# AaronWatters/contourist

Hardware: AMD Instinct MI355X
Metric: Mvoxels/s isosurface extraction on 512^3 fp32 grid (higher is better)
Workload: dtype f32

## Files before the change

contourist_amd/csrc/cx_post.h:

```cpp
#pragma once
#include <vector>

#include "cx_ctx.h"
#include "cx_dev.h"

struct cx_post_state {
    cx_buf<uint8_t> pts, prio, rep, tri, alive, parent, parent2, tkeys, tvals, flags, scan, blocksums, pts_out, tri_out, comp, misc;
    cx_buf<uint8_t> keys_out, keys_tmp, told, cls, bnd;
    cx_buf<uint8_t> ever;
    bool keys_valid = false;
    cx_buf<uint8_t> vflip;
    bool keys_edge = false, orient_live = false, vflip_valid = false;
    uint32_t orient_nt = 0;
    bool shard_mesh = false;
    double corner[3] = {1.0, 1.0, 1.0};
    uint64_t gen = 0;
    cx_buf<uint8_t> nrm[2], nrm_tmp, smap;
    int nrm_cur = 0;
    bool simplified = false, carried = false, smap_valid = false;
    bool clipped = false;
    uint32_t smap_n = 0;
    uint64_t capped_gen = 0;
    bool capped() const { return capped_gen != 0 && capped_gen == gen; }
    struct {
        bool open = false;
        uint32_t nv2 = 0, nt2 = 0;
        uint32_t nt_in = 0;
        uint32_t n1 = 0, n4 = 0, ncand = 0;
    } shard;
    cx_buf<uint8_t> mpairs, msegs, mtris, mmid, mtime, mnext;
    cx_buf<uint8_t> msegs2, mtris2, mtime2;
    cx_buf<uint8_t> meflags, metflag, menew, mecnt, medesc, me_pts, me_tri;
    void* me_pinned = nullptr;
    bool meflags_clean = false;
    uint32_t mbin_t[257] = {0}, mbin_s[257] = {0};
    double mt_lo = 0.0, mt_inv_width = 0.0;
    double mt_maxdur = 0.0, ms_maxdur = 0.0;
    bool msorted = false;
    std::vector<int64_t> me_off;
    int64_t nv_out = 0, nt_out = 0;
    int64_t ms_out = 0, mt_out = 0;
};

int cxp_state(cx_ctx* ctx, cx_post_state** out);

static inline u64 cxp_edge_table_size(size_t n) {
    u64 s = 1024;
    while (s < (5 * (u64)n) / 4 + 16) s <<= 1;
    return s;
}

int cxp_scan(cx_ctx* ctx, cx_post_state* S, const uint32_t* in, uint32_t* out, uint32_t n, uint32_t* total_dev);

int cxp_orient_pick(cx_ctx* ctx, const int32_t* tri, uint32_t nt, const double* pts, u64* parent, u64* comp, const uint32_t* keys,
                    const uint8_t* cls, uint32_t* clist, uint32_t* misc);
int cxp_orient_decide(cx_ctx* ctx, int32_t* tri, uint32_t nt, const double* pts, const u64* parent, u64* comp, const uint32_t* clist,
                      uint32_t* misc, bool wind, uint32_t* ncomp);

void cxp_iota64(hipStream_t st, u64* a, uint32_t n);
void cxp_fill64(hipStream_t st, u64* a, size_t n, u64 v);
void cxp_count_alive(hipStream_t st, const uint8_t* alive, uint32_t nt, uint32_t* counter);
void cxp_alive_u32(hipStream_t st, const uint8_t* alive, uint32_t nt, uint32_t* out);
void cxp_scan_sums(hipStream_t st, uint32_t* sums, uint32_t nb, uint32_t* total);
```

contourist_amd/csrc/cx_post.hip:

```cpp
#include <algorithm>
#include <cmath>
#include <cstring>
#include <new>
#include <string>
#include <vector>

#include "cx_post.h"

void cx_post_free(cx_ctx* ctx) {
    if (!ctx->post) return;
    cx_post_state* S = ctx->post;
    if (S->me_pinned) (void)hipHostFree(S->me_pinned);
    delete S;
    ctx->post = nullptr;
}

__global__ void cxp_k_iota64(u64* a, uint32_t n) {
    const uint32_t i = blockIdx.x * blockDim.x + threadIdx.x;
    if (i < n) a[i] = (u64)i;
}
__global__ void cxp_k_fill64(u64* a, size_t n, u64 v) {
    for (size_t i = blockIdx.x * (size_t)blockDim.x + threadIdx.x; i < n; i += (size_t)gridDim.x * blockDim.x) a[i] = v;
}
__global__ void cxp_k_jump(u64* parent, uint32_t n, uint32_t* changed) {
    const uint32_t i = blockIdx.x * blockDim.x + threadIdx.x;
    if (i >= n) return;
    u64 w = parent[i];
    uint32_t p = (uint32_t)w;
    if (p == i) return;
    bool moved = false;
#pragma unroll 1
    for (int hop = 0; hop < 3; hop++) {
        const u64 wp = parent[p];
        const uint32_t pp = (uint32_t)wp;
        if (pp == p) break;
        w = ((((w >> 32) ^ (wp >> 32)) & 1ULL) << 32) | (u64)pp;
        p = pp;
        moved = true;
    }
    if (moved) {
        parent[i] = w;
        *changed = 1u;
    }
}

#define CXP_SCAN_BLOCK 1024u
__global__ __launch_bounds__(256) void cxp_k_scan_blocks(const uint32_t* in, uint32_t* out, uint32_t* sums, uint32_t n) {
    __shared__ uint32_t s[256];
    const uint32_t base = blockIdx.x * CXP_SCAN_BLOCK + threadIdx.x * 4u;
    uint32_t v[4], t = 0;
#pragma unroll
    for (int k = 0; k < 4; k++) {
        v[k] = (base + k < n) ? in[base + k] : 0u;
        t += v[k];
    }
    s[threadIdx.x] = t;
    __syncthreads();
    for (uint32_t o = 1; o < 256; o <<= 1) {
        const uint32_t x = (threadIdx.x >= o) ? s[threadIdx.x - o] : 0u;
        __syncthreads();
        s[threadIdx.x] += x;
        __syncthreads();
    }
    uint32_t run = s[threadIdx.x] - t;
#pragma unroll
    for (int k = 0; k < 4; k++) {
        if (base + k < n) out[base + k] = run;
        run += v[k];
    }
    if (threadIdx.x == 255) sums[blockIdx.x] = s[255];
}
#define CXP_SUMS_PER_THREAD 16u
__device__ __forceinline__ void cxp_scan_sums_body(uint32_t* sums, uint32_t nb, uint32_t* total, unsigned long long* total64);
__global__ __launch_bounds__(1024) void cxp_k_scan_sums2(uint32_t* sums_a, uint32_t na, uint32_t* total_a, uint32_t* sums_b, uint32_t nb, uint32_t* total_b) {
    if (blockIdx.x == 0) cxp_scan_sums_body(sums_a, na, total_a, nullptr);
    else cxp_scan_sums_body(sums_b, nb, total_b, nullptr);
}
__global__ __launch_bounds__(1024) void cxp_k_scan_sums(uint32_t* sums, uint32_t nb, uint32_t* total, unsigned long long* total64) {
    cxp_scan_sums_body(sums, nb, total, total64);
}
__device__ __forceinline__ void cxp_scan_sums_body(uint32_t* sums, uint32_t nb, uint32_t* total, unsigned long long* total64) {
    __shared__ uint32_t s[1024];
    uint32_t carry = 0;
    unsigned long long wide = 0;
    for (uint32_t base = 0; base < nb; base += 1024u * CXP_SUMS_PER_THREAD) {
        const uint32_t i0 = base + threadIdx.x * CXP_SUMS_PER_THREAD;
        uint32_t v[CXP_SUMS_PER_THREAD], t = 0;
#pragma unroll
        for (uint32_t k = 0; k < CXP_SUMS_PER_THREAD; k++) {
            v[k] = (i0 + k < nb) ? sums[i0 + k] : 0u;
            t += v[k];
        }
        s[threadIdx.x] = t;
        __syncthreads();
        for (uint32_t o = 1; o < 1024; o <<= 1) {
            const uint32_t x = (threadIdx.x >= o) ? s[threadIdx.x - o] : 0u;
            __syncthreads();
            s[threadIdx.x] += x;
            __syncthreads();
        }
        uint32_t run = carry + s[threadIdx.x] - t;
#pragma unroll
        for (uint32_t k = 0; k < CXP_SUMS_PER_THREAD; k++) {
            if (i0 + k < nb) sums[i0 + k] = run;
            run += v[k];
        }
        const uint32_t passtot = s[1023];
        __syncthreads();
        carry += passtot;
        wide += (unsigned long long)passtot;
    }
    if (threadIdx.x == 0) {
        *total = carry;
        if (total64) *total64 = wide;
    }
}
__global__ void cxp_k_scan_add(uint32_t* out, const uint32_t* sums, uint32_t n) {
    const uint32_t i = blockIdx.x * blockDim.x + threadIdx.x;
    if (i < n) out[i] += sums[i / CXP_SCAN_BLOCK];
}

struct cxp_origin3 {
    double o[3];
};
template <int DT>
__global__ void cxp_k_vertices_f64(const cx_grid_ref A, const double* __restrict__ A64, uint32_t n1, uint32_t n2, cx_fdiv dplane, cx_fdiv drow,
                                   double value, const cx_vrec* __restrict__ verts, uint32_t nv, double* pts, uint32_t* prio, cxp_origin3 org) {
    const uint32_t v = blockIdx.x * blockDim.x + threadIdx.x;
    if (v >= nv) return;
    const uint32_t key = verts[v].x;
    const uint32_t lin = key >> 3, d = key & 7u;
    const uint32_t plane = n1 * n2;
    const uint32_t i = cx_div(lin, dplane);
    const uint32_t r = lin - i * plane;
    const uint32_t j = cx_div(r, drow);
    const uint32_t k = r - j * n2;
    const uint32_t lin2 = lin + ((d & 4u) ? plane : 0u) + ((d & 2u) ? n2 : 0u) + (d & 1u);
    const double f0 = A64 ? A64[lin] : (double)cx_sample<DT>(A, lin), f1 = A64 ? A64[lin2] : (double)cx_sample<DT>(A, lin2);
    const bool owner_low = !(f0 > f1);
    const double flow = owner_low ? f0 : f1, fhigh = owner_low ? f1 : f0;
    double ratio = 0.5;
    const double den = 1.0 * (fhigh - flow);
    if (!(fabs(den) <= 1e-8)) ratio = (value - flow) / den;
    const double q[3] = {(double)i + org.o[0], (double)j + org.o[1], (double)k + org.o[2]};
    const uint32_t db[3] = {(d >> 2) & 1u, (d >> 1) & 1u, d & 1u};
#pragma unroll
    for (int a = 0; a < 3; a++) {
        const double low = owner_low ? q[a] : q[a] + (double)db[a];
        const double high = owner_low ? q[a] + (double)db[a] : q[a];
        pts[(size_t)v * 3 + a] = low + ratio * (high - low);
    }
    prio[v] = key;
}
template <typename... Args>
static void cxp_launch_vertices_f64(dim3 grid, hipStream_t st, const cx_grid_ref& A, Args... args) {
#define CX_LAUNCH(DT) hipLaunchKernelGGL((cxp_k_vertices_f64<DT>), grid, dim3(256), 0, st, A, args...);
    CX_DISPATCH_DTYPE(A.dtype, CX_LAUNCH)
#undef CX_LAUNCH
}

__global__ void cxp_k_iota_prio(uint32_t* prio, uint32_t n) {
    const uint32_t i = blockIdx.x * blockDim.x + threadIdx.x;
    if (i < n) prio[i] = i;
}

struct cxp_weld_params {
    double ex[3];
    double thr;
};
__device__ __forceinline__ bool cxp_weld_alone(const double* p, uint32_t key, const cxp_weld_params& W) {
    if (!(W.thr > 0.0)) return false;
    const uint32_t d = key & 7u;
    const double x = (d & 4u) ? p[0] : ((d & 2u) ? p[1] : p[2]);
    const double u = x - floor(x);
    return u > W.thr && u < 1.0 - W.thr;
}
__device__ __forceinline__ u64 cxp_weld_key(const double* p, const cxp_weld_params& W) {
    const u64 q0 = (u64)((long long)(p[0] * W.ex[0]) + (1LL << 20));
    const u64 q1 = (u64)((long long)(p[1] * W.ex[1]) + (1LL << 20));
    const u64 q2 = (u64)((long long)(p[2] * W.ex[2]) + (1LL << 20));
    return (q0 << 42) | (q1 << 21) | q2;
}

__global__ void cxp_k_weld_insert(const double* pts, const uint32_t* prio, uint32_t nv, cxp_weld_params W, u64* tkeys, u64* tvals,
                                  u64 mask, const uint8_t* vkeep) {
    const uint32_t v = blockIdx.x * blockDim.x + threadIdx.x;
    if (v >= nv) return;
    if (vkeep && !vkeep[v]) return;
    if (cxp_weld_alone(pts + (size_t)v * 3, prio[v], W)) return;
    const u64 key = cxp_weld_key(pts + (size_t)v * 3, W);
    u64 slot = cxd_mix(key) & mask;
    for (;;) {
        const u64 cur = atomicCAS(&tkeys[slot], CXD_EMPTY, key);
        if (cur == CXD_EMPTY || cur == key) break;
        slot = (slot + 1) & mask;
    }
    atomicMax(&tvals[slot], ((u64)prio[v] << 32) | (u64)v);
}
__global__ void cxp_k_weld_lookup(const double* pts, uint32_t nv, cxp_weld_params W, const u64* tkeys, const u64* tvals, u64 mask,
                                  uint32_t* rep, const uint8_t* vkeep, const uint32_t* prio) {
    const uint32_t v = blockIdx.x * blockDim.x + threadIdx.x;
    if (v >= nv) return;
    if (vkeep && !vkeep[v]) { rep[v] = v; return; }
    if (cxp_weld_alone(pts + (size_t)v * 3, prio[v], W)) { rep[v] = v; return; }
    const u64 key = cxp_weld_key(pts + (size_t)v * 3, W);
    u64 slot = cxd_mix(key) & mask;
    while (tkeys[slot] != key) slot = (slot + 1) & mask;
    rep[v] = (uint32_t)tvals[slot];
}

__global__ void cxp_k_remap(int32_t* tri, uint8_t* alive, uint32_t nt, const uint32_t* map, const u64* parent, uint8_t* involved = nullptr,
                            uint8_t* ever = nullptr) {
    const uint32_t t = blockIdx.x * blockDim.x + threadIdx.x;
    if (t >= nt || !alive[t]) return;
    const uint32_t x[3] = {(uint32_t)tri[(size_t)t * 3], (uint32_t)tri[(size_t)t * 3 + 1], (uint32_t)tri[(size_t)t * 3 + 2]};
    uint32_t v[3];
    if (map) {
        v[0] = map[x[0]]; v[1] = map[x[1]]; v[2] = map[x[2]];
    } else {
        uint32_t par;
#pragma unroll
        for (int s = 0; s < 3; s++) v[s] = cxp_find(parent, x[s], par);
    }
#pragma unroll
    for (int s = 0; s < 3; s++) {
        if (v[s] != x[s]) {
            tri[(size_t)t * 3 + s] = (int32_t)v[s];
            if (involved) involved[v[s]] = 1;
            if (ever) ever[v[s]] = 1;
        }
    }
    if (v[0] == v[1] || v[0] == v[2] || v[1] == v[2]) alive[t] = 0;
}

struct cxp_tri3 {
    uint32_t a, b, c;
};
__device__ __forceinline__ cxp_tri3 cxp_sorted3(uint32_t x, uint32_t y, uint32_t z) {
    if (x > y) { const uint32_t t = x; x = y; y = t; }
    if (y > z) { const uint32_t t = y; y = z; z = t; }
    if (x > y) { const uint32_t t = x; x = y; y = t; }
    cxp_tri3 r = {x, y, z};
    return r;
}
__device__ __forceinline__ bool cxp_less3(const cxp_tri3& p, const cxp_tri3& q) {
    if (p.a != q.a) return p.a < q.a;
    if (p.b != q.b) return p.b < q.b;
    return p.c < q.c;
}

__global__ void cxp_k_dedupe_insert(const int32_t* tri, const uint32_t* tprio3, const uint8_t* alive, uint32_t nt, u64* table,
                                    u64 mask, const uint8_t* involved = nullptr) {
    const uint32_t t = blockIdx.x * blockDim.x + threadIdx.x;
    if (t >= nt || !alive[t]) return;
    if (involved && !(involved[tri[(size_t)t * 3]] | involved[tri[(size_t)t * 3 + 1]] | involved[tri[(size_t)t * 3 + 2]])) return;
    const cxp_tri3 me = cxp_sorted3((uint32_t)tri[(size_t)t * 3], (uint32_t)tri[(size_t)t * 3 + 1], (uint32_t)tri[(size_t)t * 3 + 2]);
    const cxp_tri3 mp = {tprio3[(size_t)t * 3], tprio3[(size_t)t * 3 + 1], tprio3[(size_t)t * 3 + 2]};
    u64 slot = cxd_mix(((u64)me.a << 40) ^ ((u64)me.b << 20) ^ (u64)me.c ^ ((u64)me.c << 50)) & mask;
    for (;;) {
        u64 cur = atomicCAS(&table[slot], CXD_EMPTY, (u64)t);
        if (cur == CXD_EMPTY) return;
        for (;;) {
            const uint32_t o = (uint32_t)cur;
            const cxp_tri3 ot = cxp_sorted3((uint32_t)tri[(size_t)o * 3], (uint32_t)tri[(size_t)o * 3 + 1], (uint32_t)tri[(size_t)o * 3 + 2]);
            if (ot.a != me.a || ot.b != me.b || ot.c != me.c) break;
            const cxp_tri3 op = {tprio3[(size_t)o * 3], tprio3[(size_t)o * 3 + 1], tprio3[(size_t)o * 3 + 2]};
            if (!cxp_less3(mp, op)) return;
            const u64 seen = atomicCAS(&table[slot], cur, (u64)t);
            if (seen == cur) return;
            cur = seen;
        }
        slot = (slot + 1) & mask;
    }
}
__global__ void cxp_k_dedupe_resolve(const int32_t* tri, uint8_t* alive, uint32_t nt, const u64* table, u64 mask, const uint8_t* involved = nullptr) {
    const uint32_t t = blockIdx.x * blockDim.x + threadIdx.x;
    if (t >= nt || !alive[t]) return;
    if (involved && !(involved[tri[(size_t)t * 3]] | involved[tri[(size_t)t * 3 + 1]] | involved[tri[(size_t)t * 3 + 2]])) return;
    const cxp_tri3 me = cxp_sorted3((uint32_t)tri[(size_t)t * 3], (uint32_t)tri[(size_t)t * 3 + 1], (uint32_t)tri[(size_t)t * 3 + 2]);
    u64 slot = cxd_mix(((u64)me.a << 40) ^ ((u64)me.b << 20) ^ (u64)me.c ^ ((u64)me.c << 50)) & mask;
    for (;;) {
        const uint32_t o = (uint32_t)table[slot];
        if (o == t) return;
        const cxp_tri3 ot = cxp_sorted3((uint32_t)tri[(size_t)o * 3], (uint32_t)tri[(size_t)o * 3 + 1], (uint32_t)tri[(size_t)o * 3 + 2]);
        if (ot.a == me.a && ot.b == me.b && ot.c == me.c) { alive[t] = 0; return; }
        slot = (slot + 1) & mask;
    }
}

__global__ void cxp_k_tri_prio(const int32_t* tri, const uint32_t* prio, uint32_t nt, uint32_t* tprio3) {
    const uint32_t t = blockIdx.x * blockDim.x + threadIdx.x;
    if (t >= nt) return;
    const cxp_tri3 p = cxp_sorted3(prio[tri[(size_t)t * 3]], prio[tri[(size_t)t * 3 + 1]], prio[tri[(size_t)t * 3 + 2]]);
    tprio3[(size_t)t * 3] = p.a; tprio3[(size_t)t * 3 + 1] = p.b; tprio3[(size_t)t * 3 + 2] = p.c;
}

__global__ __launch_bounds__(256) void cxp_k_count_alive(const uint8_t* alive, uint32_t nt, uint32_t* counter) {
    __shared__ uint32_t s_n;
    if (threadIdx.x == 0) s_n = 0;
    __syncthreads();
    uint32_t n = 0;
    for (uint32_t t = blockIdx.x * blockDim.x + threadIdx.x; t < nt; t += gridDim.x * blockDim.x) n += alive[t] ? 1u : 0u;
#pragma unroll
    for (int o = 32; o > 0; o >>= 1) n += (uint32_t)__shfl_xor((int)n, o);
    if ((threadIdx.x & 63u) == 0 && n) atomicAdd(&s_n, n);
    __syncthreads();
    if (threadIdx.x == 0 && s_n) atomicAdd(counter, s_n);
}

__global__ void cxp_k_tiny(const int32_t* tri, uint8_t* alive, uint32_t nt, const double* pts, double ic0, double ic1, double ic2,
                           double eps, u64* parent, const uint32_t* prio, uint8_t* moved) {
    const uint32_t t = blockIdx.x * blockDim.x + threadIdx.x;
    if (t >= nt || !alive[t]) return;
    const uint32_t v0 = tri[(size_t)t * 3], v1 = tri[(size_t)t * 3 + 1], v2 = tri[(size_t)t * 3 + 2];
    const double ic[3] = {ic0, ic1, ic2};
    double worst = 0.0;
#pragma unroll
    for (int a = 0; a < 3; a++) {
        const double x0 = pts[(size_t)v0 * 3 + a], x1 = pts[(size_t)v1 * 3 + a], x2 = pts[(size_t)v2 * 3 + a];
        const double d = (fmax(x0, fmax(x1, x2)) - fmin(x0, fmin(x1, x2))) * ic[a];
        worst = fmax(worst, d);
    }
    if (worst < eps) {
        alive[t] = 0;
        cxp_union(parent, prio, v0, v1, 0);
        cxp_union(parent, prio, v0, v2, 0);
        moved[v0] = moved[v1] = moved[v2] = 1;
    }
}
__global__ void cxp_k_move(double* pts, const double* pts_src, const u64* parent, const uint8_t* moved, uint32_t nv) {
    const uint32_t v = blockIdx.x * blockDim.x + threadIdx.x;
    if (v >= nv || !moved[v]) return;
    uint32_t par;
    const uint32_t r = cxp_find(parent, v, par);
#pragma unroll
    for (int a = 0; a < 3; a++) pts[(size_t)v * 3 + a] = pts_src[(size_t)r * 3 + a];
}

__global__ void cxp_k_degenerate(const int32_t* tri, uint8_t* alive, uint32_t nt, const double* pts, u64* parent, const uint32_t* prio) {
    const uint32_t t = blockIdx.x * blockDim.x + threadIdx.x;
    if (t >= nt || !alive[t]) return;
    const uint32_t v[3] = {(uint32_t)tri[(size_t)t * 3], (uint32_t)tri[(size_t)t * 3 + 1], (uint32_t)tri[(size_t)t * 3 + 2]};
    double P[3][3];
#pragma unroll
    for (int s = 0; s < 3; s++)
#pragma unroll
        for (int a = 0; a < 3; a++) P[s][a] = pts[(size_t)v[s] * 3 + a];
    const double ux = P[0][0] - P[2][0], uy = P[0][1] - P[2][1], uz = P[0][2] - P[2][2];
    const double wx = P[1][0] - P[2][0], wy = P[1][1] - P[2][1], wz = P[1][2] - P[2][2];
    const double cx = uy * wz - uz * wy, cy = uz * wx - ux * wz, cz = ux * wy - uy * wx;
    if (fabs(cx) <= 1e-8 && fabs(cy) <= 1e-8 && fabs(cz) <= 1e-8) {
        alive[t] = 0;
        const int pr[3][2] = {{0, 1}, {0, 2}, {1, 2}};
#pragma unroll
        for (int e = 0; e < 3; e++) {
            const int i = pr[e][0], j = pr[e][1];
            bool close = true;
#pragma unroll
            for (int a = 0; a < 3; a++) close = close && (fabs(P[i][a] - P[j][a]) <= 1e-8 + 1e-5 * fabs(P[j][a]));
            if (close) cxp_union(parent, prio, v[i], v[j], 0);
        }
    }
}

__global__ void cxp_k_alive_u32(const uint8_t* alive, uint32_t nt, uint32_t* out) {
    const uint32_t t = blockIdx.x * blockDim.x + threadIdx.x;
    if (t < nt) out[t] = alive[t] ? 1u : 0u;
}
__device__ __forceinline__ uint32_t cxp_block_excl4(const uint32_t v[4], uint32_t* s, uint32_t& block_total) {
    const uint32_t t = v[0] + v[1] + v[2] + v[3];
    s[threadIdx.x] = t;
    __syncthreads();
    for (uint32_t o = 1; o < 256; o <<= 1) {
        const uint32_t x = (threadIdx.x >= o) ? s[threadIdx.x - o] : 0u;
        __syncthreads();
        s[threadIdx.x] += x;
        __syncthreads();
    }
    block_total = s[255];
    return s[threadIdx.x] - t;
}
__global__ __launch_bounds__(256) void cxp_k_me_count(const uint8_t* flags, uint32_t n, uint32_t* count) {
    __shared__ uint32_t s_n;
    if (threadIdx.x == 0) s_n = 0;
    __syncthreads();
    const uint32_t base = blockIdx.x * CXP_SCAN_BLOCK + threadIdx.x * 4u;
    uint32_t c = 0;
    if (base + 3u < n) {
        const uint32_t w = *reinterpret_cast<const uint32_t*>(flags + base);
        c = __popc(w & 0x01010101u);
    } else {
        for (uint32_t k = 0; k < 4 && base + k < n; k++) c += flags[base + k] ? 1u : 0u;
    }
#pragma unroll
    for (int o = 32; o > 0; o >>= 1) c += (uint32_t)__shfl_xor((int)c, o);
    if ((threadIdx.x & 63u) == 0 && c) atomicAdd(&s_n, c);
    __syncthreads();
    if (threadIdx.x == 0) count[blockIdx.x] = s_n;
}
__global__ void cxp_k_mark_used8(const int32_t* tri, const uint8_t* alive, uint32_t nt, uint8_t* used) {
    const uint32_t t = blockIdx.x * blockDim.x + threadIdx.x;
    if (t >= nt || !alive[t]) return;
    const uint32_t a = (uint32_t)tri[(size_t)t * 3], b = (uint32_t)tri[(size_t)t * 3 + 1], c = (uint32_t)tri[(size_t)t * 3 + 2];
    used[a] = 1; used[b] = 1; used[c] = 1;
}
__global__ __launch_bounds__(256) void cxp_k_compact_pts_fused(const double* pts, const uint8_t* used, const uint32_t* voff, uint32_t nv, uint32_t* vnew,
                                                               double* out, const uint32_t* keys, uint32_t* keys_out, const uint8_t* ever, uint8_t* ever_out) {
    __shared__ uint32_t s[256];
    const uint32_t base = blockIdx.x * CXP_SCAN_BLOCK + threadIdx.x * 4u;
    uint32_t f[4];
#pragma unroll
    for (uint32_t k = 0; k < 4; k++) f[k] = (base + k < nv && used[base + k]) ? 1u : 0u;
    uint32_t tot;
    uint32_t id = voff[blockIdx.x] + cxp_block_excl4(f, s, tot);
    if (tot == 0u) return;
#pragma unroll
    for (uint32_t k = 0; k < 4; k++) {
        if (!f[k]) continue;
        const uint32_t v = base + k;
        const double x = pts[(size_t)v * 3], y = pts[(size_t)v * 3 + 1], z = pts[(size_t)v * 3 + 2];
        const uint32_t key = keys_out ? keys[v] : 0u;
        const uint8_t e = ever_out ? ever[v] : (uint8_t)0;
        vnew[v] = id;
        out[(size_t)id * 3] = x; out[(size_t)id * 3 + 1] = y; out[(size_t)id * 3 + 2] = z;
        if (keys_out) keys_out[id] = key;
        if (ever_out) ever_out[id] = e;
        id++;
    }
}
__global__ __launch_bounds__(256) void cxp_k_compact_tri_fused(const int32_t* tri, const uint8_t* alive, const uint32_t* toff, const uint32_t* vnew, uint32_t nt,
                                                               int32_t* out, uint32_t* told) {
    __shared__ uint32_t s[256];
    const uint32_t base = blockIdx.x * CXP_SCAN_BLOCK + threadIdx.x * 4u;
    uint32_t f[4];
#pragma unroll
    for (uint32_t k = 0; k < 4; k++) f[k] = (base + k < nt && alive[base + k]) ? 1u : 0u;
    uint32_t tot;
    uint32_t id = toff[blockIdx.x] + cxp_block_excl4(f, s, tot);
    if (tot == 0u) return;
#pragma unroll
    for (uint32_t k = 0; k < 4; k++) {
        if (!f[k]) continue;
        const uint32_t t = base + k;
        const uint32_t a = (uint32_t)tri[(size_t)t * 3], b = (uint32_t)tri[(size_t)t * 3 + 1], c = (uint32_t)tri[(size_t)t * 3 + 2];
        const uint32_t na = vnew[a], nb = vnew[b], nc = vnew[c];
        out[(size_t)id * 3] = (int32_t)na; out[(size_t)id * 3 + 1] = (int32_t)nb; out[(size_t)id * 3 + 2] = (int32_t)nc;
        if (told) told[id] = t;
        id++;
    }
}

__device__ __forceinline__ uint32_t cxp_edge_dir(const int32_t* tri, uint32_t t, uint32_t lo, uint32_t hi) {
    const uint32_t a = tri[(size_t)t * 3], b = tri[(size_t)t * 3 + 1], c = tri[(size_t)t * 3 + 2];
    return ((a == lo && b == hi) || (b == lo && c == hi) || (c == lo && a == hi)) ? 1u : 0u;
}
__global__ void cxp_k_edges_claim(const int32_t* tri, uint32_t nt, u64* tab, u64 mask, u64 mult) {
    const uint32_t t = blockIdx.x * blockDim.x + threadIdx.x;
    if (t >= nt) return;
    const uint32_t v[3] = {(uint32_t)tri[(size_t)t * 3], (uint32_t)tri[(size_t)t * 3 + 1], (uint32_t)tri[(size_t)t * 3 + 2]};
    for (int e = 0; e < 3; e++) {
        const uint32_t p = v[e], q = v[(e + 1) % 3];
        const uint32_t lo = min(p, q), hi = max(p, q);
        const u64 key = ((u64)lo << 32) | (u64)hi;
        u64 slot = cxp_edge_slot(lo, hi, mask, mult);
        for (;;) {
            u64 cur = __hip_atomic_load(&tab[2 * slot], __ATOMIC_RELAXED, __HIP_MEMORY_SCOPE_AGENT);
            if (cur == CXD_EMPTY) cur = atomicCAS(&tab[2 * slot], CXD_EMPTY, key);
            if (cur == CXD_EMPTY) { __hip_atomic_store(&tab[2 * slot + 1], (u64)t, __ATOMIC_RELAXED, __HIP_MEMORY_SCOPE_AGENT); break; }
            if (cur == key) break;
            slot = (slot + 1) & mask;
        }
    }
}
__global__ void cxp_k_edges_link(const int32_t* tri, uint32_t nt, const u64* tab, u64 mask, u64 mult, u64* parent, int coherent) {
    const uint32_t t = blockIdx.x * blockDim.x + threadIdx.x;
    if (t >= nt) return;
    const uint32_t v[3] = {(uint32_t)tri[(size_t)t * 3], (uint32_t)tri[(size_t)t * 3 + 1], (uint32_t)tri[(size_t)t * 3 + 2]};
#pragma unroll
    for (int e = 0; e < 3; e++) {
        const uint32_t p = v[e], q = v[(e + 1) % 3];
        const uint32_t lo = min(p, q), hi = max(p, q);
        const u64 key = ((u64)lo << 32) | (u64)hi;
        u64 slot = cxp_edge_slot(lo, hi, mask, mult);
        while (tab[2 * slot] != key) slot = (slot + 1) & mask;
        const uint32_t o = (uint32_t)tab[2 * slot + 1];
        if (o == t) continue;
        uint32_t rel = 0;
        if (!coherent) rel = (cxp_edge_dir(tri, t, lo, hi) == cxp_edge_dir(tri, o, lo, hi)) ? 1u : 0u;
        cxp_union(parent, nullptr, t, o, rel);
    }
}
#ifndef CXP_LINK_BLOCK
#define CXP_LINK_BLOCK 2048u
#endif
#define CXP_LINK_PER_THREAD (CXP_LINK_BLOCK / 256u)
__device__ __forceinline__ uint32_t cxp_lfind(uint32_t* lp, uint32_t x) {
    for (;;) {
        const uint32_t p = ((volatile uint32_t*)lp)[x];
        if (p == x) return x;
        const uint32_t g = ((volatile uint32_t*)lp)[p];
        if (g != p) ((volatile uint32_t*)lp)[x] = g;
        x = p;
    }
}
__global__ __launch_bounds__(256) void cxp_k_edges_link_local(const int32_t* tri, uint32_t nt, const u64* tab, u64 mask, u64 mult, u64* parent,
                                                              uint32_t* others) {
    __shared__ uint32_t lp[CXP_LINK_BLOCK];
    const uint32_t b0 = blockIdx.x * CXP_LINK_BLOCK;
    for (uint32_t x = threadIdx.x; x < CXP_LINK_BLOCK; x += 256u) lp[x] = x;
    __syncthreads();
#pragma unroll 1
    for (uint32_t i = 0; i < CXP_LINK_PER_THREAD; i++) {
        const uint32_t t = b0 + i * 256u + threadIdx.x;
        if (t >= nt) continue;
        const uint32_t v[3] = {(uint32_t)tri[(size_t)t * 3], (uint32_t)tri[(size_t)t * 3 + 1], (uint32_t)tri[(size_t)t * 3 + 2]};
#pragma unroll
        for (int e = 0; e < 3; e++) {
            const uint32_t p = v[e], q = v[(e + 1) % 3];
            const uint32_t lo = min(p, q), hi = max(p, q);
            const u64 key = ((u64)lo << 32) | (u64)hi;
            u64 slot = cxp_edge_slot(lo, hi, mask, mult);
            while (tab[2 * slot] != key) slot = (slot + 1) & mask;
            const uint32_t o = (uint32_t)tab[2 * slot + 1];
            uint32_t far = CXD_NONE;
            if (o != t) {
                if (o - b0 < CXP_LINK_BLOCK) {
                    uint32_t a = t - b0, b = o - b0;
                    for (;;) {
                        a = cxp_lfind(lp, a);
                        b = cxp_lfind(lp, b);
                        if (a == b) break;
                        const uint32_t win = min(a, b), lose = max(a, b);
                        if (atomicCAS(&lp[lose], lose, win) == lose) break;
                    }
                } else {
                    far = o;
                }
            }
            others[(size_t)t * 3 + e] = far;
        }
    }
    __syncthreads();
    for (uint32_t i = 0; i < CXP_LINK_PER_THREAD; i++) {
        const uint32_t x = i * 256u + threadIdx.x;
        if (b0 + x >= nt) continue;
        const uint32_t r = cxp_lfind(lp, x);
        if (r != x) parent[b0 + x] = (u64)(b0 + r);
    }
}
__global__ void cxp_k_edges_link_cross(uint32_t nt, const uint32_t* others, u64* parent) {
    const uint32_t t = blockIdx.x * blockDim.x + threadIdx.x;
    if (t >= nt) return;
#pragma unroll
    for (int e = 0; e < 3; e++) {
        const uint32_t o = others[(size_t)t * 3 + e];
        if (o != CXD_NONE) cxp_union0(parent, t, o);
    }
}
#ifndef CXP_EB
#define CXP_EB 512u
#endif
#define CXP_EB_PER (CXP_EB / 256u)
#define CXP_EB_SLOTS (4u * CXP_EB)
__global__ __launch_bounds__(256) void cxp_k_edges_block(const int32_t* tri, uint32_t nt, const uint8_t* ever, u64* tab, u64 mask, u64 mult,
                                                         u64* parent, uint8_t* others, uint32_t probe_limit, uint32_t* overflow) {
    __shared__ u64 lkey[CXP_EB_SLOTS];
    __shared__ uint16_t lfirst[CXP_EB_SLOTS];
    __shared__ uint8_t lpair[CXP_EB_SLOTS];
    __shared__ uint32_t lp[CXP_EB];
    const uint32_t b0 = blockIdx.x * CXP_EB;
    for (uint32_t x = threadIdx.x; x < CXP_EB_SLOTS; x += 256u) { lkey[x] = CXD_EMPTY; lpair[x] = 0; }
    for (uint32_t x = threadIdx.x; x < CXP_EB; x += 256u) lp[x] = x;
    uint32_t lo_[CXP_EB_PER][3], hi_[CXP_EB_PER][3];
    uint32_t flag_[CXP_EB_PER][3];
    uint16_t slot_[CXP_EB_PER][3];
#pragma unroll
    for (uint32_t i = 0; i < CXP_EB_PER; i++) {
        const uint32_t t = min(b0 + i * 256u + threadIdx.x, nt - 1u);
        const uint32_t v[3] = {(uint32_t)tri[(size_t)t * 3], (uint32_t)tri[(size_t)t * 3 + 1], (uint32_t)tri[(size_t)t * 3 + 2]};
#pragma unroll
        for (int e = 0; e < 3; e++) {
            lo_[i][e] = min(v[e], v[(e + 1) % 3]);
            hi_[i][e] = max(v[e], v[(e + 1) % 3]);
        }
    }
#pragma unroll
    for (uint32_t i = 0; i < CXP_EB_PER; i++)
#pragma unroll
        for (int e = 0; e < 3; e++) flag_[i][e] = (uint32_t)ever[lo_[i][e]] | (uint32_t)ever[hi_[i][e]];
    __syncthreads();
#pragma unroll
    for (uint32_t i = 0; i < CXP_EB_PER; i++) {
        const uint32_t lt = i * 256u + threadIdx.x;
        if (b0 + lt >= nt) continue;
#pragma unroll
        for (int e = 0; e < 3; e++) {
            const u64 key = ((u64)lo_[i][e] << 32) | (u64)hi_[i][e];
            uint32_t slot = (uint32_t)cxd_mix(key) & (CXP_EB_SLOTS - 1u);
            for (uint32_t probes = 0; probes < CXP_EB_SLOTS; probes++) {
                const u64 cur = atomicCAS((unsigned long long*)&lkey[slot], (unsigned long long)CXD_EMPTY, (unsigned long long)key);
                if (cur == CXD_EMPTY) { lfirst[slot] = (uint16_t)lt; break; }
                if (cur == key) break;
                slot = (slot + 1u) & (CXP_EB_SLOTS - 1u);
            }
            slot_[i][e] = (uint16_t)slot;
        }
    }
    __syncthreads();
#pragma unroll
    for (uint32_t i = 0; i < CXP_EB_PER; i++) {
        const uint32_t lt = i * 256u + threadIdx.x;
        if (b0 + lt >= nt) continue;
#pragma unroll
        for (int e = 0; e < 3; e++) {
            const uint32_t first = lfirst[slot_[i][e]];
            if (first == lt) continue;
            lpair[slot_[i][e]] = 1;
            uint32_t a = lt, b = first;
            for (;;) {
                a = cxp_lfind(lp, a);
                b = cxp_lfind(lp, b);
                if (a == b) break;
                const uint32_t win = min(a, b), lose = max(a, b);
                if (atomicCAS(&lp[lose], lose, win) == lose) break;
            }
        }
    }
    __syncthreads();
#pragma unroll
    for (uint32_t i = 0; i < CXP_EB_PER; i++) {
        const uint32_t lt = i * 256u + threadIdx.x, t = b0 + lt;
        if (t >= nt) continue;
        uint32_t farbits = 0;
#pragma unroll
        for (int e = 0; e < 3; e++) {
            const uint32_t lo = lo_[i][e], hi = hi_[i][e];
            const bool taker = lfirst[slot_[i][e]] == lt;
            if (taker && (flag_[i][e] != 0u || !lpair[slot_[i][e]])) {
                farbits |= 1u << e;
                const u64 key = ((u64)lo << 32) | (u64)hi;
                u64 slot = cxp_edge_slot(lo, hi, mask, mult);
                for (uint32_t probes = 0;; probes++) {
                    if (probes >= probe_limit) { *overflow = 1u; break; }
                    u64 cur = __hip_atomic_load(&tab[2 * slot], __ATOMIC_RELAXED, __HIP_MEMORY_SCOPE_AGENT);
                    if (cur == CXD_EMPTY) cur = atomicCAS(&tab[2 * slot], CXD_EMPTY, key);
                    if (cur == CXD_EMPTY) { __hip_atomic_store(&tab[2 * slot + 1], (u64)t, __ATOMIC_RELAXED, __HIP_MEMORY_SCOPE_AGENT); break; }
                    if (cur == key) break;
                    slot = (slot + 1) & mask;
                }
            }
        }
        others[t] = (uint8_t)farbits;
    }
    for (uint32_t x = threadIdx.x; x < CXP_EB; x += 256u) {
        if (b0 + x >= nt) continue;
        const uint32_t r = cxp_lfind(lp, x);
        if (r != x) parent[b0 + x] = (u64)(b0 + r);
    }
}
__global__ void cxp_k_edges_link_far(const int32_t* tri, uint32_t nt, const u64* tab, u64 mask, u64 mult, const uint8_t* others, u64* parent) {
    const uint32_t t = blockIdx.x * blockDim.x + threadIdx.x;
    if (t >= nt) return;
    const uint32_t fb = others[t];
    if (!fb) return;
    const uint32_t v[3] = {(uint32_t)tri[(size_t)t * 3], (uint32_t)tri[(size_t)t * 3 + 1], (uint32_t)tri[(size_t)t * 3 + 2]};
#pragma unroll
    for (int e = 0; e < 3; e++) {
        if (!((fb >> e) & 1u)) continue;
        const uint32_t p = v[e], q = v[(e + 1) % 3];
        const uint32_t lo = min(p, q), hi = max(p, q);
        const u64 key = ((u64)lo << 32) | (u64)hi;
        u64 slot = cxp_edge_slot(lo, hi, mask, mult);
        while (tab[2 * slot] != key) slot = (slot + 1) & mask;
        const uint32_t o = (uint32_t)tab[2 * slot + 1];
        if (o != t) cxp_union0(parent, t, o);
    }
}
#define CXP_OWN(cls, t) (!(cls) || (cls)[t] <= 2u)
__global__ void cxp_k_comp_maxx(const int32_t* tri, uint32_t nt, const double* pts, const u64* parent, u64* cmaxx, const uint8_t* cls) {
    const uint32_t idx = blockIdx.x * blockDim.x + threadIdx.x;
    const uint32_t t = nt - 1u - idx;
    const bool have = idx < nt && CXP_OWN(cls, t);
    uint32_t root = 0;
    u64 m = 0;
    if (have) {
        root = (uint32_t)parent[t];
#pragma unroll
        for (int s = 0; s < 3; s++) m = max(m, cxd_orderable(pts[(size_t)tri[(size_t)t * 3 + s] * 3]));
    }
    cxp_wave_max64(cmaxx, root, m, have);
}
__global__ void cxp_k_comp_list(const int32_t* tri, uint32_t nt, const double* pts, const u64* parent, const u64* cmaxx, const uint8_t* cls,
                                uint32_t* list, uint32_t* nlist) {
    const uint32_t t = blockIdx.x * blockDim.x + threadIdx.x;
    bool hit = false;
    if (t < nt && CXP_OWN(cls, t)) {
        const u64 m = cmaxx[(uint32_t)parent[t]];
#pragma unroll
        for (int s = 0; s < 3; s++) hit = hit || cxd_orderable(pts[(size_t)tri[(size_t)t * 3 + s] * 3]) == m;
    }
    const uint64_t hits = __ballot(hit);
    if (hits == 0ULL) return;
    const uint32_t lane = threadIdx.x & 63u;
    uint32_t base = 0;
    if (lane == (uint32_t)(__ffsll((long long)hits) - 1)) base = atomicAdd(nlist, (uint32_t)__popcll(hits));
    base = (uint32_t)__shfl((int)base, __ffsll((long long)hits) - 1);
    if (hit) list[base + (uint32_t)__popcll(hits & ((1ULL << lane) - 1ULL))] = t;
}
#define CXP_FOR_TRI(t)                                                                                                   \
    for (uint32_t i_ = blockIdx.x * blockDim.x + threadIdx.x, n_ = list ? *nlist : nt; i_ < n_; i_ += gridDim.x * blockDim.x) { \
        const uint32_t t = list ? list[i_] : i_;
#define CXP_END_FOR }
__global__ void cxp_k_comp_maxv(const int32_t* tri, uint32_t nt, const double* pts, const u64* parent, const u64* cmaxx, u64* cmaxv,
                                const uint32_t* keys, const uint8_t* cls, const uint32_t* list, const uint32_t* nlist) {
    CXP_FOR_TRI(t)
        if (!CXP_OWN(cls, t)) continue;
        const uint32_t root = (uint32_t)parent[t];
        const u64 m = cmaxx[root];
#pragma unroll
        for (int s = 0; s < 3; s++) {
            const uint32_t v = tri[(size_t)t * 3 + s];
            if (cxd_orderable(pts[(size_t)v * 3]) == m) cxd_max64(&cmaxv[root], ((u64)(keys ? keys[v] : v) << 32) | (u64)v);
        }
    CXP_END_FOR
}
__device__ __forceinline__ double cxp_dotx(const int32_t* tri, uint32_t t, const double* pts) {
    const uint32_t a = tri[(size_t)t * 3], b = tri[(size_t)t * 3 + 1], c = tri[(size_t)t * 3 + 2];
    const double aby = pts[(size_t)a * 3 + 1] - pts[(size_t)b * 3 + 1], abz = pts[(size_t)a * 3 + 2] - pts[(size_t)b * 3 + 2];
    const double acy = pts[(size_t)a * 3 + 1] - pts[(size_t)c * 3 + 1], acz = pts[(size_t)a * 3 + 2] - pts[(size_t)c * 3 + 2];
    return aby * acz - abz * acy;
}
__global__ void cxp_k_comp_start(const int32_t* tri, uint32_t nt, const double* pts, const u64* parent, const u64* cmaxv,
                                 u64* cbest, const uint8_t* cls, const uint32_t* list, const uint32_t* nlist) {
    CXP_FOR_TRI(t)
        if (!CXP_OWN(cls, t)) continue;
        const uint32_t root = (uint32_t)parent[t];
        const uint32_t vm = (uint32_t)cmaxv[root];
        if ((uint32_t)tri[(size_t)t * 3] != vm && (uint32_t)tri[(size_t)t * 3 + 1] != vm && (uint32_t)tri[(size_t)t * 3 + 2] != vm) continue;
        cxd_max64(&cbest[root], cxd_orderable(fabs(cxp_dotx(tri, t, pts))));
    CXP_END_FOR
}
__global__ void cxp_k_comp_pick(const int32_t* tri, uint32_t nt, const double* pts, const u64* parent, const u64* cmaxv,
                                const u64* cbest, uint32_t* cstart, const uint8_t* cls, const uint32_t* list, const uint32_t* nlist) {
    CXP_FOR_TRI(t)
        if (!CXP_OWN(cls, t)) continue;
        const uint32_t root = (uint32_t)parent[t];
        const uint32_t vm = (uint32_t)cmaxv[root];
        if ((uint32_t)tri[(size_t)t * 3] != vm && (uint32_t)tri[(size_t)t * 3 + 1] != vm && (uint32_t)tri[(size_t)t * 3 + 2] != vm) continue;
        if (cxd_orderable(fabs(cxp_dotx(tri, t, pts))) == cbest[root]) cxd_max32(&cstart[root], t);
    CXP_END_FOR
}
__global__ void cxp_k_comp_decide(const int32_t* tri, uint32_t nt, const double* pts, const u64* parent, const uint32_t* cstart, u64* cflip,
                                  const uint32_t* list, const uint32_t* nlist) {
    CXP_FOR_TRI(t)
        const u64 w = parent[t];
        const uint32_t root = (uint32_t)w;
        if (cstart[root] != t) continue;
        const uint32_t spar = (uint32_t)(w >> 32) & 1u;
        cflip[root] = (u64)((((cxp_dotx(tri, t, pts) < 0.0) ? 1u : 0u) ^ spar) & 1u);
    CXP_END_FOR
}
__global__ void cxp_k_orient(int32_t* tri, uint32_t nt, const u64* parent, const u64* cflip, uint32_t* ncomp) {
    const uint32_t t = blockIdx.x * blockDim.x + threadIdx.x;
    if (t >= nt) return;
    const u64 w = parent[t];
    const uint32_t root = (uint32_t)w, par = (uint32_t)(w >> 32) & 1u;
    if (root == t) atomicAdd(ncomp, 1u);
    if ((par ^ (uint32_t)cflip[root]) & 1u) {
        const int32_t a = tri[(size_t)t * 3];
        tri[(size_t)t * 3] = tri[(size_t)t * 3 + 2];
        tri[(size_t)t * 3 + 2] = a;
    }
}

struct cxp_shard {
    uint32_t plane;
    uint32_t own_lo, own_hi;
    uint32_t layers;
};
__global__ void cxp_k_shard_classify(const uint32_t* tprio3, uint8_t* alive, uint32_t nt, cxp_shard sh, cx_fdiv dplane, uint8_t* cls,
                                     uint32_t* counts) {
    const uint32_t t = blockIdx.x * blockDim.x + threadIdx.x;
    if (t >= nt) return;
    uint8_t c = 255;
    if (alive[t]) {
        const uint32_t layer = cx_div(tprio3[(size_t)t * 3] >> 3, dplane);
        if (layer >= sh.own_lo && layer < sh.own_hi) {
            c = 0;
            if (layer == sh.own_lo && sh.own_lo > 0u) c = 1;
            else if (layer + 1u == sh.own_hi && sh.own_hi < sh.layers) c = 2;
        } else if (layer + 1u == sh.own_lo) c = 3;
        else if (layer == sh.own_hi) c = 4;
        if (c == 255) alive[t] = 0;
        else if (c == 1) atomicAdd(&counts[0], 1u);
        else if (c == 4) atomicAdd(&counts[1], 1u);
    }
    cls[t] = c;
}
__global__ void cxp_k_shard_gather_cls(const uint8_t* cls, const uint32_t* told, uint32_t nt2, uint8_t* cls2) {
    const uint32_t t = blockIdx.x * blockDim.x + threadIdx.x;
    if (t < nt2) cls2[t] = cls[told[t]];
}
__device__ __forceinline__ u64 cxp_triple_hash(u64 a, u64 b, u64 c) {
    u64 h = cxd_mix(a + 0x9E3779B97F4A7C15ULL);
    h = cxd_mix(h ^ (b + 0xC2B2AE3D27D4EB4FULL));
    return cxd_mix(h ^ (c + 0x165667B19E3779F9ULL));
}
__global__ void cxp_k_shard_boundary(const uint8_t* cls2, const uint32_t* told, const uint32_t* tprio3, const u64* parent, uint32_t nt2,
                                     u64 key_offset, uint32_t* counters, uint32_t cap1, uint32_t cap4, u64* hash1, uint32_t* label1,
                                     u64* hash4, uint32_t* label4, uint8_t* open) {
    const uint32_t t = blockIdx.x * blockDim.x + threadIdx.x;
    if (t >= nt2) return;
    const uint32_t c = cls2[t];
    if (c != 1u && c != 4u) return;
    const uint32_t root = (uint32_t)parent[t];
    open[root] = 1;
    const uint32_t o = told[t];
    const u64 h = cxp_triple_hash((u64)tprio3[(size_t)o * 3] + key_offset, (u64)tprio3[(size_t)o * 3 + 1] + key_offset,
                                  (u64)tprio3[(size_t)o * 3 + 2] + key_offset);
    if (c == 1u) {
        const uint32_t at = atomicAdd(&counters[0], 1u);
        if (at < cap1) { hash1[at] = h; label1[at] = root; }
    } else {
        const uint32_t at = atomicAdd(&counters[1], 1u);
        if (at < cap4) { hash4[at] = h; label4[at] = root; }
    }
}
struct cxp_cand { double x, nx; uint32_t label, vkey, sign, has; };
__global__ void cxp_k_shard_candidates(const int32_t* tri2, const double* pts2, const uint32_t* keys2, const u64* parent, const uint8_t* open,
                                       uint32_t nt2, const u64* cmaxx, const u64* cmaxv, const uint32_t* cstart, uint32_t* counter,
                                       uint32_t cap, cxp_cand* out) {
    const uint32_t t = blockIdx.x * blockDim.x + threadIdx.x;
    if (t >= nt2 || (uint32_t)parent[t] != t || !open[t]) return;
    const uint32_t at = atomicAdd(counter, 1u);
    if (at >= cap) return;
    cxp_cand c;
    c.label = t; c.has = cmaxx[t] != 0 ? 1u : 0u; c.x = 0.0; c.nx = 0.0; c.vkey = 0; c.sign = 0;
    if (c.has) {
        const uint32_t vm = (uint32_t)cmaxv[t];
        const double d = cxp_dotx(tri2, cstart[t], pts2);
        c.x = pts2[(size_t)vm * 3]; c.vkey = keys2[vm]; c.nx = fabs(d); c.sign = d < 0.0 ? 1u : 0u;
    }
    out[at] = c;
}
__global__ void cxp_k_shard_set_flips(const uint32_t* labels, const uint8_t* flips, uint32_t n, uint32_t nt2, u64* cflip) {
    const uint32_t i = blockIdx.x * blockDim.x + threadIdx.x;
    if (i < n && labels[i] < nt2) cflip[labels[i]] = (u64)(flips[i] & 1u);
}
__global__ void cxp_k_shard_own_alive(const uint8_t* cls2, uint32_t nt2, uint8_t* alive) {
    const uint32_t t = blockIdx.x * blockDim.x + threadIdx.x;
    if (t < nt2) alive[t] = cls2[t] <= 2u ? 1 : 0;
}


void cxp_iota64(hipStream_t st, u64* a, uint32_t n) {
    hipLaunchKernelGGL(cxp_k_iota64, dim3(cx_blocks(n)), dim3(256), 0, st, a, n);
}
void cxp_fill64(hipStream_t st, u64* a, size_t n, u64 v) {
    hipLaunchKernelGGL(cxp_k_fill64, dim3(2048), dim3(256), 0, st, a, n, v);
}
void cxp_count_alive(hipStream_t st, const uint8_t* alive, uint32_t nt, uint32_t* counter) {
    hipLaunchKernelGGL(cxp_k_count_alive, dim3(std::min(cx_blocks(nt), 1024u)), dim3(256), 0, st, alive, nt, counter);
}
void cxp_alive_u32(hipStream_t st, const uint8_t* alive, uint32_t nt, uint32_t* out) {
    hipLaunchKernelGGL(cxp_k_alive_u32, dim3(cx_blocks(nt)), dim3(256), 0, st, alive, nt, out);
}
void cxp_scan_sums(hipStream_t st, uint32_t* sums, uint32_t nb, uint32_t* total) {
    hipLaunchKernelGGL(cxp_k_scan_sums, dim3(1), dim3(1024), 0, st, sums, nb, total, (unsigned long long*)nullptr);
}

int cxp_scan(cx_ctx* ctx, cx_post_state* S, const uint32_t* in, uint32_t* out, uint32_t n, uint32_t* total_dev) {
    const uint32_t nb = cx_blocks(n, CXP_SCAN_BLOCK);
    int rc = S->blocksums.grow(ctx, (size_t)(nb + 1) * sizeof(uint32_t));
    if (rc) return rc;
    uint32_t* sums = S->blocksums.as<uint32_t>();
    hipLaunchKernelGGL(cxp_k_scan_blocks, dim3(nb ? nb : 1), dim3(256), 0, ctx->stream, in, out, sums, n);
    hipLaunchKernelGGL(cxp_k_scan_sums, dim3(1), dim3(1024), 0, ctx->stream, sums, nb, total_dev, (unsigned long long*)nullptr);
    hipLaunchKernelGGL(cxp_k_scan_add, dim3(cx_blocks(n)), dim3(256), 0, ctx->stream, out, sums, n);
    return CX_OK;
}

int cx_scan_u32(cx_ctx* ctx, const uint32_t* in, uint32_t* out, uint32_t n, uint32_t* sums_tmp, uint32_t* total_dev, unsigned long long* total64_dev) {
    const uint32_t nb = cx_blocks(n, CXP_SCAN_BLOCK);
    hipLaunchKernelGGL(cxp_k_scan_blocks, dim3(nb ? nb : 1), dim3(256), 0, ctx->stream, in, out, sums_tmp, n);
    hipLaunchKernelGGL(cxp_k_scan_sums, dim3(1), dim3(1024), 0, ctx->stream, sums_tmp, nb, total_dev, total64_dev);
    if (n) hipLaunchKernelGGL(cxp_k_scan_add, dim3(cx_blocks(n)), dim3(256), 0, ctx->stream, out, sums_tmp, n);
    return CX_OK;
}

static int cxp_flatten(cx_ctx* ctx, u64* parent, uint32_t n, uint32_t* changed_dev) {
    for (int it = 0; it < 64; it++) {
        CX_HIP(ctx, hipMemsetAsync(changed_dev, 0, sizeof(uint32_t), ctx->stream));
        hipLaunchKernelGGL(cxp_k_jump, dim3(cx_blocks(n)), dim3(256), 0, ctx->stream, parent, n, changed_dev);
        uint32_t changed = 0;
        CX_HIP(ctx, hipMemcpyAsync(&changed, changed_dev, sizeof(uint32_t), hipMemcpyDeviceToHost, ctx->stream));
        CX_HIP(ctx, hipStreamSynchronize(ctx->stream));
        if (!changed) return CX_OK;
    }
    ctx->err = "union-find did not flatten";
    return CX_ERR_HIP;
}

int cxp_orient_pick(cx_ctx* ctx, const int32_t* tri, uint32_t nt, const double* pts, u64* parent, u64* comp, const uint32_t* keys,
                    const uint8_t* cls, uint32_t* clist, uint32_t* misc) {
    int rc;
    hipStream_t st = ctx->stream;
    u64* cmaxx = comp;
    u64* cbest = cmaxx + nt;
    u64* cmaxv = cbest + nt;
    uint32_t* cstart = (uint32_t*)(cmaxv + nt);
    if ((rc = cxp_flatten(ctx, parent, nt, misc))) return rc;
    CX_HIP(ctx, hipMemsetAsync(cmaxx, 0, (size_t)nt * (3 * sizeof(u64) + sizeof(uint32_t)), st));
    CX_HIP(ctx, hipMemsetAsync(misc + 3, 0, sizeof(uint32_t), st));
    hipLaunchKernelGGL(cxp_k_comp_maxx, dim3(cx_blocks(nt)), dim3(256), 0, st, tri, nt, pts, parent, cmaxx, cls);
    const uint32_t* cn = misc + 11;
    const dim3 lgrid(std::min(cx_blocks(nt), 1024u));
    CX_HIP(ctx, hipMemsetAsync(misc + 11, 0, sizeof(uint32_t), st));
    hipLaunchKernelGGL(cxp_k_comp_list, dim3(cx_blocks(nt)), dim3(256), 0, st, tri, nt, pts, parent, cmaxx, cls, clist, misc + 11);
    hipLaunchKernelGGL(cxp_k_comp_maxv, lgrid, dim3(256), 0, st, tri, nt, pts, parent, cmaxx, cmaxv, keys, cls, (const uint32_t*)clist, cn);
    hipLaunchKernelGGL(cxp_k_comp_start, lgrid, dim3(256), 0, st, tri, nt, pts, parent, cmaxv, cbest, cls, (const uint32_t*)clist, cn);
    hipLaunchKernelGGL(cxp_k_comp_pick, lgrid, dim3(256), 0, st, tri, nt, pts, parent, cmaxv, cbest, cstart, cls, (const uint32_t*)clist, cn);
    return CX_OK;
}
int cxp_orient_decide(cx_ctx* ctx, int32_t* tri, uint32_t nt, const double* pts, const u64* parent, u64* comp, const uint32_t* clist,
                      uint32_t* misc, bool wind, uint32_t* ncomp) {
    hipStream_t st = ctx->stream;
    u64* cbest = comp + nt;
    const uint32_t* cstart = (const uint32_t*)(comp + 3 * (size_t)nt);
    const uint32_t* cn = misc + 11;
    const dim3 lgrid(std::min(cx_blocks(nt), 1024u));
    hipLaunchKernelGGL(cxp_k_comp_decide, lgrid, dim3(256), 0, st, tri, nt, pts, parent, cstart, cbest, clist, cn);
    if (wind) {
        hipLaunchKernelGGL(cxp_k_orient, dim3(cx_blocks(nt)), dim3(256), 0, st, tri, nt, parent, cbest, misc + 3);
        CX_HIP(ctx, hipMemcpyAsync(ncomp, misc + 3, sizeof(uint32_t), hipMemcpyDeviceToHost, st));
    }
    return CX_OK;
}

static int cxp_clean_orient(cx_ctx* ctx, cx_post_state* S, uint32_t nv, uint32_t nt, bool do_clean, bool do_orient,
                            uint32_t* tprio3, int64_t* out_counts, bool coherent, uint8_t* involved = nullptr, const cxp_shard* shard = nullptr,
                            uint8_t* ever = nullptr) {
    int rc;
    double* pts = S->pts.as<double>();
    uint32_t* prio = S->prio.as<uint32_t>();
    int32_t* tri = S->tri.as<int32_t>();
    uint8_t* alive = S->alive.as<uint8_t>();
    uint32_t* misc = S->misc.as<uint32_t>();
    hipStream_t st = ctx->stream;
    S->keys_valid = false;
    S->keys_edge = false; S->orient_live = false; S->vflip_valid = false;
    S->shard_mesh = false; S->gen++; S->orient_nt = 0;
    S->shard.open = false;
    S->simplified = false; S->carried = false; S->smap_valid = false; S->clipped = false;
    if (do_clean && nt) {
        u64* parent2 = S->parent2.as<u64>();
        hipLaunchKernelGGL(cxp_k_iota64, dim3(cx_blocks(nv)), dim3(256), 0, st, parent2, nv);
        hipLaunchKernelGGL(cxp_k_degenerate, dim3(cx_blocks(nt)), dim3(256), 0, st, tri, alive, nt, pts, parent2, prio);
        if (involved) CX_HIP(ctx, hipMemsetAsync(involved, 0, nv, st));
        hipLaunchKernelGGL(cxp_k_remap, dim3(cx_blocks(nt)), dim3(256), 0, st, tri, alive, nt, (const uint32_t*)nullptr, parent2, involved, ever);
        const u64 tsz = involved ? cxp_edge_table_size(nt) : cx_table_size(nt);
        if ((rc = S->tkeys.grow(ctx, tsz * sizeof(u64)))) return rc;
        hipLaunchKernelGGL(cxp_k_fill64, dim3(2048), dim3(256), 0, st, S->tkeys.as<u64>(), (size_t)tsz, CXD_EMPTY);
        hipLaunchKernelGGL(cxp_k_dedupe_insert, dim3(cx_blocks(nt)), dim3(256), 0, st, tri, tprio3, alive, nt, S->tkeys.as<u64>(), tsz - 1, (const uint8_t*)involved);
        hipLaunchKernelGGL(cxp_k_dedupe_resolve, dim3(cx_blocks(nt)), dim3(256), 0, st, tri, alive, nt, S->tkeys.as<u64>(), tsz - 1, (const uint8_t*)involved);
    }
    uint8_t* cls = nullptr;
    uint32_t* told = nullptr;
    if (shard) {
        if ((rc = S->cls.grow(ctx, 3 * (size_t)nt + 64))) return rc;
        if ((rc = S->told.grow(ctx, ((size_t)nt + 16) * sizeof(uint32_t)))) return rc;
        cls = S->cls.as<uint8_t>();
        told = S->told.as<uint32_t>();
        CX_HIP(ctx, hipMemsetAsync(misc + 6, 0, 2 * sizeof(uint32_t), st));
        if (nt) hipLaunchKernelGGL(cxp_k_shard_classify, dim3(cx_blocks(nt)), dim3(256), 0, st, tprio3, alive, nt, *shard, cx_fdiv_make(shard->plane), cls, misc + 6);
    }
    if ((rc = S->flags.grow(ctx, (size_t)(nv + nt + 16) * sizeof(uint32_t)))) return rc;
    if ((rc = S->scan.grow(ctx, (size_t)(nv + 16) * sizeof(uint32_t)))) return rc;
    const uint32_t nbv = cx_blocks(nv, CXP_SCAN_BLOCK), nbt = cx_blocks(nt, CXP_SCAN_BLOCK);
    if ((rc = S->blocksums.grow(ctx, (size_t)(nbv + nbt + 16) * sizeof(uint32_t)))) return rc;
    uint8_t* used = S->flags.as<uint8_t>();
    uint32_t* vnew = S->scan.as<uint32_t>();
    uint32_t* voff = S->blocksums.as<uint32_t>();
    uint32_t* toff = voff + nbv + 8;
    uint32_t nv2 = 0, nt2 = 0;
    if (nt) {
        CX_HIP(ctx, hipMemsetAsync(used, 0, (size_t)nv, st));
        hipLaunchKernelGGL(cxp_k_mark_used8, dim3(cx_blocks(nt)), dim3(256), 0, st, tri, alive, nt, used);
        hipLaunchKernelGGL(cxp_k_me_count, dim3(nbv), dim3(256), 0, st, (const uint8_t*)used, nv, voff);
        hipLaunchKernelGGL(cxp_k_me_count, dim3(nbt), dim3(256), 0, st, (const uint8_t*)alive, nt, toff);
        hipLaunchKernelGGL(cxp_k_scan_sums2, dim3(2), dim3(1024), 0, st, voff, nbv, misc + 1, toff, nbt, misc + 2);
        uint32_t h[2];
        CX_HIP(ctx, hipMemcpyAsync(h, misc + 1, 2 * sizeof(uint32_t), hipMemcpyDeviceToHost, st));
        CX_HIP(ctx, hipStreamSynchronize(st));
        nv2 = h[0]; nt2 = h[1];
    }
    if ((rc = S->pts_out.grow(ctx, (size_t)(nv2 + 1) * 3 * sizeof(double)))) return rc;
    if ((rc = S->tri_out.grow(ctx, (size_t)(nt2 + 1) * 3 * sizeof(int32_t)))) return rc;
    if ((rc = S->keys_out.grow(ctx, (size_t)(nv2 + 1) * sizeof(uint32_t)))) return rc;
    double* pts2 = S->pts_out.as<double>();
    int32_t* tri2 = S->tri_out.as<int32_t>();
    uint32_t* keys2 = S->keys_out.as<uint32_t>();
    if (nt2) {
        hipLaunchKernelGGL(cxp_k_compact_pts_fused, dim3(nbv), dim3(256), 0, st, (const double*)pts, (const uint8_t*)used, (const uint32_t*)voff, nv, vnew, pts2,
                           (const uint32_t*)prio, keys2, (const uint8_t*)ever, ever ? ever + nv : nullptr);
        hipLaunchKernelGGL(cxp_k_compact_tri_fused, dim3(nbt), dim3(256), 0, st, (const int32_t*)tri, (const uint8_t*)alive, (const uint32_t*)toff,
                           (const uint32_t*)vnew, nt, tri2, told);
    }
    S->nv_out = nv2; S->nt_out = nt2;
    S->keys_valid = true;
    uint8_t* cls2 = nullptr;
    if (shard) {
        cls2 = cls + nt;
        if (nt2) hipLaunchKernelGGL(cxp_k_shard_gather_cls, dim3(cx_blocks(nt2)), dim3(256), 0, st, cls, told, nt2, cls2);
    }
    uint32_t ncomp = 0;
    if (do_orient && nt2) {
        const u64 esz_full = cxp_edge_table_size((size_t)nt2 * 3);
        const bool blocks = ever && coherent && !cx_debug_knob("CX_LINK_GLOBAL", 0);
        u64 esz = esz_full;
        if (blocks && !cx_debug_knob("CX_EDGE_TABLE_FULL", 0)) {
            esz = 1024;
            while (esz < (u64)nt2 + 16) esz <<= 1;
            if (cx_debug_knob("CX_EDGE_TABLE_TINY", 0)) esz = 1024;
            if (esz > esz_full) esz = esz_full;
        }
        if ((rc = S->parent.grow(ctx, (size_t)nt2 * sizeof(u64)))) return rc;
        if ((rc = S->comp.grow(ctx, (size_t)nt2 * (3 * sizeof(u64) + sizeof(uint32_t))))) return rc;
        u64* parent = S->parent.as<u64>();
        u64* cmaxx = S->comp.as<u64>();
        u64* cbest = cmaxx + nt2;
        u64* cmaxv = cbest + nt2;
        uint32_t* cstart = (uint32_t*)(cmaxv + nt2);
        uint32_t* others = S->comp.as<uint32_t>();
        for (;;) {
            if ((rc = S->tkeys.grow(ctx, 2 * esz * sizeof(u64)))) return rc;
            u64* etab = S->tkeys.as<u64>();
            hipLaunchKernelGGL(cxp_k_fill64, dim3(2048), dim3(256), 0, st, etab, (size_t)(2 * esz), CXD_EMPTY);
            hipLaunchKernelGGL(cxp_k_iota64, dim3(cx_blocks(nt2)), dim3(256), 0, st, parent, nt2);
            const u64 emult = (blocks && esz != esz_full) ? 0 : std::max<u64>(1, esz / std::max<u64>(1, (u64)nv2));
            if (blocks) {
                CX_HIP(ctx, hipMemsetAsync(misc + 12, 0, sizeof(uint32_t), st));
                hipLaunchKernelGGL(cxp_k_edges_block, dim3((nt2 + CXP_EB - 1u) / CXP_EB), dim3(256), 0, st, tri2, nt2, (const uint8_t*)(ever + nv), etab, esz - 1,
                                   emult, parent, (uint8_t*)others, esz == esz_full ? 0xFFFFFFFFu : 256u, misc + 12);
                if (esz != esz_full) {
                    uint32_t over = 0;
                    CX_HIP(ctx, hipMemcpyAsync(&over, misc + 12, sizeof(uint32_t), hipMemcpyDeviceToHost, st));
                    CX_HIP(ctx, hipStreamSynchronize(st));
                    if (over) { esz = esz_full; continue; }
                }
                hipLaunchKernelGGL(cxp_k_edges_link_far, dim3(cx_blocks(nt2)), dim3(256), 0, st, tri2, nt2, etab, esz - 1, emult, (const uint8_t*)others, parent);
            } else {
                hipLaunchKernelGGL(cxp_k_edges_claim, dim3(cx_blocks(nt2)), dim3(256), 0, st, tri2, nt2, etab, esz - 1, emult);
                if (coherent && !cx_debug_knob("CX_LINK_ONE_STEP", 0)) {
                    hipLaunchKernelGGL(cxp_k_edges_link_local, dim3((nt2 + CXP_LINK_BLOCK - 1u) / CXP_LINK_BLOCK), dim3(256), 0, st, tri2, nt2, etab, esz - 1,
                                       emult, parent, others);
                    hipLaunchKernelGGL(cxp_k_edges_link_cross, dim3(cx_blocks(nt2)), dim3(256), 0, st, nt2, others, parent);
                } else
                    hipLaunchKernelGGL(cxp_k_edges_link, dim3(cx_blocks(nt2)), dim3(256), 0, st, tri2, nt2, etab, esz - 1, emult, parent, coherent ? 1 : 0);
            }
            break;
        }
        uint32_t* clist = S->flags.as<uint32_t>();
        if ((rc = cxp_orient_pick(ctx, tri2, nt2, pts2, parent, cmaxx, keys2, cls2, clist, misc))) return rc;
        if (shard) {
            uint32_t hb[2] = {0, 0};
            CX_HIP(ctx, hipMemcpyAsync(hb, misc + 6, 2 * sizeof(uint32_t), hipMemcpyDeviceToHost, st));
            CX_HIP(ctx, hipStreamSynchronize(st));
            const size_t n1 = hb[0], n4 = hb[1], nb = n1 + n4;
            if ((rc = S->bnd.grow(ctx, (nb + 2) * (sizeof(u64) + sizeof(cxp_cand) + sizeof(uint32_t)) + 64))) return rc;
            u64* hash1 = S->bnd.as<u64>();
            u64* hash4 = hash1 + n1;
            cxp_cand* cand = (cxp_cand*)(hash4 + n4);
            uint32_t* label1 = (uint32_t*)(cand + nb);
            uint32_t* label4 = label1 + n1;
            uint8_t* open = cls + 2 * (size_t)nt;
            CX_HIP(ctx, hipMemsetAsync(open, 0, nt2, st));
            CX_HIP(ctx, hipMemsetAsync(misc + 8, 0, 3 * sizeof(uint32_t), st));
            if (nb) {
                const u64 key_offset = ((u64)ctx->origin[0] * (u64)shard->plane) << 3;
                hipLaunchKernelGGL(cxp_k_shard_boundary, dim3(cx_blocks(nt2)), dim3(256), 0, st, cls2, told, tprio3, parent, nt2, key_offset, misc + 8,
                                   (uint32_t)n1, (uint32_t)n4, hash1, label1, hash4, label4, open);
                hipLaunchKernelGGL(cxp_k_shard_candidates, dim3(cx_blocks(nt2)), dim3(256), 0, st, tri2, pts2, keys2, parent, open, nt2, cmaxx, cmaxv,
                                   cstart, misc + 10, (uint32_t)nb, cand);
            }
            uint32_t h2[3] = {0, 0, 0};
            CX_HIP(ctx, hipMemcpyAsync(h2, misc + 8, 3 * sizeof(uint32_t), hipMemcpyDeviceToHost, st));
            CX_HIP(ctx, hipStreamSynchronize(st));
            if (h2[0] != n1 || h2[1] != n4 || h2[2] > nb) { ctx->err = "sharded Level 1: boundary lists do not add up"; return CX_ERR_HIP; }
            S->shard.n1 = (uint32_t)n1; S->shard.n4 = (uint32_t)n4; S->shard.ncand = h2[2];
        }
        if ((rc = cxp_orient_decide(ctx, tri2, nt2, pts2, parent, cmaxx, clist, misc, !shard, &ncomp))) return rc;
        if (!shard) { S->orient_live = true; S->orient_nt = nt2; }
        CX_HIP(ctx, hipStreamSynchronize(st));
    } else if (shard) {
        S->shard.n1 = 0; S->shard.n4 = 0; S->shard.ncand = 0;
    }
    if (shard) { S->shard.open = true; S->shard.nv2 = nv2; S->shard.nt2 = nt2; S->shard.nt_in = nt; }
    CX_HIP(ctx, hipGetLastError());
    if (out_counts) {
        out_counts[0] = nv2; out_counts[1] = nt2; out_counts[4] = ncomp;
    }
    return CX_OK;
}

static int cxp_shard_finish(cx_ctx* ctx, cx_post_state* S, const uint32_t* labels, const uint8_t* flips, uint32_t n, int64_t* out_counts) {
    int rc;
    hipStream_t st = ctx->stream;
    uint32_t* misc = S->misc.as<uint32_t>();
    const uint32_t nv2 = S->shard.nv2, nt2 = S->shard.nt2;
    S->shard.open = false;
    uint32_t ncomp = 0, nv3 = 0, nt3 = 0;
    if (nt2) {
        u64* parent = S->parent.as<u64>();
        u64* cflip = S->comp.as<u64>() + nt2;
        int32_t* tri2 = S->tri_out.as<int32_t>();
        const uint8_t* cls2 = S->cls.as<const uint8_t>() + S->shard.nt_in;
        if (n) {
            if ((rc = S->keys_tmp.grow(ctx, std::max((size_t)n * 5 + 64, (size_t)(nv2 + 1) * sizeof(uint32_t))))) return rc;
            uint32_t* dl = S->keys_tmp.as<uint32_t>();
            uint8_t* df = (uint8_t*)(dl + n);
            CX_HIP(ctx, hipMemcpyAsync(dl, labels, (size_t)n * sizeof(uint32_t), hipMemcpyHostToDevice, st));
            CX_HIP(ctx, hipMemcpyAsync(df, flips, (size_t)n, hipMemcpyHostToDevice, st));
            hipLaunchKernelGGL(cxp_k_shard_set_flips, dim3(cx_blocks(n)), dim3(256), 0, st, dl, df, n, nt2, cflip);
        }
        CX_HIP(ctx, hipMemsetAsync(misc + 3, 0, sizeof(uint32_t), st));
        hipLaunchKernelGGL(cxp_k_orient, dim3(cx_blocks(nt2)), dim3(256), 0, st, tri2, nt2, parent, cflip, misc + 3);
        uint8_t* alive = S->alive.as<uint8_t>();
        uint8_t* used = S->flags.as<uint8_t>();
        uint32_t* vnew = S->scan.as<uint32_t>();
        const uint32_t nbv = cx_blocks(nv2, CXP_SCAN_BLOCK), nbt = cx_blocks(nt2, CXP_SCAN_BLOCK);
        if ((rc = S->blocksums.grow(ctx, (size_t)(nbv + nbt + 16) * sizeof(uint32_t)))) return rc;
        uint32_t* voff = S->blocksums.as<uint32_t>();
        uint32_t* toff = voff + nbv + 8;
        hipLaunchKernelGGL(cxp_k_shard_own_alive, dim3(cx_blocks(nt2)), dim3(256), 0, st, cls2, nt2, alive);
        CX_HIP(ctx, hipMemsetAsync(used, 0, (size_t)nv2, st));
        hipLaunchKernelGGL(cxp_k_mark_used8, dim3(cx_blocks(nt2)), dim3(256), 0, st, (const int32_t*)tri2, (const uint8_t*)alive, nt2, used);
        hipLaunchKernelGGL(cxp_k_me_count, dim3(nbv), dim3(256), 0, st, (const uint8_t*)used, nv2, voff);
        hipLaunchKernelGGL(cxp_k_me_count, dim3(nbt), dim3(256), 0, st, (const uint8_t*)alive, nt2, toff);
        hipLaunchKernelGGL(cxp_k_scan_sums2, dim3(2), dim3(1024), 0, st, voff, nbv, misc + 1, toff, nbt, misc + 2);
        uint32_t h[3];
        CX_HIP(ctx, hipMemcpyAsync(h, misc + 1, 3 * sizeof(uint32_t), hipMemcpyDeviceToHost, st));
        CX_HIP(ctx, hipStreamSynchronize(st));
        nv3 = h[0]; nt3 = h[1]; ncomp = h[2];
        if ((rc = S->pts.grow(ctx, (size_t)(nv3 + 1) * 3 * sizeof(double)))) return rc;
        if ((rc = S->tri.grow(ctx, (size_t)(nt3 + 1) * 3 * sizeof(int32_t)))) return rc;
        if ((rc = S->keys_tmp.grow(ctx, (size_t)(nv3 + 1) * sizeof(uint32_t)))) return rc;
        if (nt3) {
            hipLaunchKernelGGL(cxp_k_compact_pts_fused, dim3(nbv), dim3(256), 0, st, S->pts_out.as<const double>(), (const uint8_t*)used, (const uint32_t*)voff, nv2, vnew,
                               S->pts.as<double>(), S->keys_out.as<const uint32_t>(), S->keys_tmp.as<uint32_t>(), (const uint8_t*)nullptr, (uint8_t*)nullptr);
            hipLaunchKernelGGL(cxp_k_compact_tri_fused, dim3(nbt), dim3(256), 0, st, (const int32_t*)tri2, (const uint8_t*)alive, (const uint32_t*)toff,
                               (const uint32_t*)vnew, nt2, S->tri.as<int32_t>(), (uint32_t*)nullptr);
        }
        if (nt3) {
            CX_HIP(ctx, hipMemcpyAsync(S->pts_out.get(), S->pts.get(), (size_t)nv3 * 3 * sizeof(double), hipMemcpyDeviceToDevice, st));
            CX_HIP(ctx, hipMemcpyAsync(S->tri_out.get(), S->tri.get(), (size_t)nt3 * 3 * sizeof(int32_t), hipMemcpyDeviceToDevice, st));
            CX_HIP(ctx, hipMemcpyAsync(S->keys_out.get(), S->keys_tmp.get(), (size_t)nv3 * sizeof(uint32_t), hipMemcpyDeviceToDevice, st));
        }
        CX_HIP(ctx, hipStreamSynchronize(st));
    }
    S->nv_out = nv3; S->nt_out = nt3;
    S->keys_valid = true;
    S->shard_mesh = true; S->gen++;
    CX_HIP(ctx, hipGetLastError());
    if (out_counts) { out_counts[0] = nv3; out_counts[1] = nt3; out_counts[4] = ncomp; }
    return CX_OK;
}

int cxp_state(cx_ctx* ctx, cx_post_state** out) {
    if (!ctx->post) ctx->post = new (std::nothrow) cx_post_state();
    if (!ctx->post) return CX_ERR_NOMEM;
    *out = ctx->post;
    ctx->post->ms_out = 0; ctx->post->mt_out = 0; ctx->post->msorted = false; ctx->post->me_off.clear();
    return ctx->post->misc.grow(ctx, 512 * sizeof(uint32_t));
}

__global__ void cxp_k_unique_edges(const int32_t* tri, const uint8_t* alive, uint32_t nt, u64* ekeys, u64 mask) {
    const uint32_t t = blockIdx.x * blockDim.x + threadIdx.x;
    if (t >= nt || !alive[t]) return;
    const uint32_t v[3] = {(uint32_t)tri[(size_t)t * 3], (uint32_t)tri[(size_t)t * 3 + 1], (uint32_t)tri[(size_t)t * 3 + 2]};
    for (int e = 0; e < 3; e++) {
        const uint32_t p = v[e], q = v[(e + 1) % 3];
        const u64 key = ((u64)min(p, q) << 32) | (u64)max(p, q);
        u64 slot = cxd_mix(key) & mask;
        for (;;) {
            u64 cur = __hip_atomic_load(&ekeys[slot], __ATOMIC_RELAXED, __HIP_MEMORY_SCOPE_AGENT);
            if (cur == CXD_EMPTY) cur = atomicCAS(&ekeys[slot], CXD_EMPTY, key);
            if (cur == CXD_EMPTY || cur == key) break;
            slot = (slot + 1) & mask;
        }
    }
}
__global__ void cxp_k_smooth_accumulate(const u64* ekeys, size_t n, const double* pts, double* sum, uint32_t* cnt) {
    const size_t i = blockIdx.x * (size_t)blockDim.x + threadIdx.x;
    if (i >= n || ekeys[i] == CXD_EMPTY) return;
    const uint32_t a = (uint32_t)(ekeys[i] >> 32), b = (uint32_t)ekeys[i];
#pragma unroll
    for (int c = 0; c < 3; c++) {
        atomicAdd(&sum[(size_t)a * 3 + c], pts[(size_t)b * 3 + c]);
        atomicAdd(&sum[(size_t)b * 3 + c], pts[(size_t)a * 3 + c]);
    }
    atomicAdd(&cnt[a], 1u);
    atomicAdd(&cnt[b], 1u);
}
#define CXP_SM_SLOTS 1024u
__global__ __launch_bounds__(256) void cxp_k_smooth_edges(const int32_t* tri, const uint8_t* alive, uint32_t nt, u64* ekeys, u64 mask, const double* pts,
                                                          double* sum, uint32_t* cnt) {
    __shared__ uint32_t lv[CXP_SM_SLOTS];
    __shared__ uint32_t lc[CXP_SM_SLOTS];
    __shared__ double ls[CXP_SM_SLOTS][3];
    for (uint32_t x = threadIdx.x; x < CXP_SM_SLOTS; x += 256u) { lv[x] = CXD_NONE; lc[x] = 0u; ls[x][0] = 0.0; ls[x][1] = 0.0; ls[x][2] = 0.0; }
    __syncthreads();
    const uint32_t t = blockIdx.x * blockDim.x + threadIdx.x;
    if (t < nt && alive[t]) {
        const uint32_t v[3] = {(uint32_t)tri[(size_t)t * 3], (uint32_t)tri[(size_t)t * 3 + 1], (uint32_t)tri[(size_t)t * 3 + 2]};
        auto add = [&](uint32_t to, uint32_t from) {
            uint32_t slot = (to * 0x9E3779B1u) >> 22;
            for (;;) {
                const uint32_t cur = atomicCAS(&lv[slot], CXD_NONE, to);
                if (cur == CXD_NONE || cur == to) break;
                slot = (slot + 1u) & (CXP_SM_SLOTS - 1u);
            }
            unsafeAtomicAdd(&ls[slot][0], pts[(size_t)from * 3]);
            unsafeAtomicAdd(&ls[slot][1], pts[(size_t)from * 3 + 1]);
            unsafeAtomicAdd(&ls[slot][2], pts[(size_t)from * 3 + 2]);
            atomicAdd(&lc[slot], 1u);
        };
        for (int e = 0; e < 3; e++) {
            const uint32_t p = v[e], q = v[(e + 1) % 3];
            const u64 key = ((u64)min(p, q) << 32) | (u64)max(p, q);
            u64 slot = cxd_mix(key) & mask;
            bool mine = false;
            for (;;) {
                u64 cur = __hip_atomic_load(&ekeys[slot], __ATOMIC_RELAXED, __HIP_MEMORY_SCOPE_AGENT);
                if (cur == CXD_EMPTY) { cur = atomicCAS(&ekeys[slot], CXD_EMPTY, key); mine = cur == CXD_EMPTY; }
                if (cur == CXD_EMPTY || cur == key) break;
                slot = (slot + 1) & mask;
            }
            if (mine && p != q) { add(p, q); add(q, p); }
            else if (mine) { add(p, p); add(p, p); }
        }
    }
    __syncthreads();
    for (uint32_t x = threadIdx.x; x < CXP_SM_SLOTS; x += 256u) {
        const uint32_t to = lv[x];
        if (to == CXD_NONE) continue;
        atomicAdd(&sum[(size_t)to * 3], ls[x][0]);
        atomicAdd(&sum[(size_t)to * 3 + 1], ls[x][1]);
        atomicAdd(&sum[(size_t)to * 3 + 2], ls[x][2]);
        atomicAdd(&cnt[to], lc[x]);
    }
}
__global__ void cxp_k_smooth_apply(double* pts, const double* sum, const uint32_t* cnt, uint32_t nv, double factor) {
    const uint32_t v = blockIdx.x * blockDim.x + threadIdx.x;
    if (v >= nv || cnt[v] == 0u) return;
    const double inv = 1.0 / (double)(cnt[v] + 1u);
#pragma unroll
    for (int c = 0; c < 3; c++) {
        const double p = pts[(size_t)v * 3 + c];
        const double avg = (sum[(size_t)v * 3 + c] + p) * inv;
        pts[(size_t)v * 3 + c] = p - factor * (p - avg);
    }
}

extern "C" int cx_postprocess3d_ex(cx_ctx* ctx, uint32_t flags, double smooth, int64_t* out_counts);

extern "C" int cx_postprocess3d(cx_ctx* ctx, uint32_t flags, int64_t* out_counts) {
    return cx_postprocess3d_ex(ctx, flags, 0.0, out_counts);
}

static int cxp_reserve3d(cx_ctx* ctx, cx_post_state* S, uint32_t nv, uint32_t nt) {
    int rc;
    if ((rc = S->pts.grow(ctx, (size_t)(nv + 1) * 3 * sizeof(double)))) return rc;
    if ((rc = S->prio.grow(ctx, (size_t)(nv + 1) * sizeof(uint32_t)))) return rc;
    if ((rc = S->rep.grow(ctx, (size_t)(nv + 1) * (sizeof(uint32_t) + 1)))) return rc;
    if ((rc = S->tri.grow(ctx, (size_t)(nt + 1) * 3 * sizeof(int32_t) * 2))) return rc;
    if ((rc = S->alive.grow(ctx, (size_t)nt + 16))) return rc;
    if ((rc = S->parent.grow(ctx, (size_t)(nv + 1) * sizeof(u64)))) return rc;
    if ((rc = S->parent2.grow(ctx, (size_t)(nv + 1) * sizeof(u64)))) return rc;
    return CX_OK;
}
static int cxp_run3d(cx_ctx* ctx, cx_post_state* S, uint32_t nv, uint32_t nt, const double corner[3], const uint8_t* vkeep, bool do_clean,
                     double smooth, bool coherent, int64_t* counts, bool edge_crossings = false, const cxp_shard* shard = nullptr, bool march_mesh = false) {
    int rc;
    hipStream_t st = ctx->stream;
    double* pts = S->pts.as<double>();
    uint32_t* prio = S->prio.as<uint32_t>();
    uint32_t* rep = S->rep.as<uint32_t>();
    uint8_t* moved = (uint8_t*)(rep + nv + 1);
    int32_t* tri = S->tri.as<int32_t>();
    uint32_t* tprio3 = (uint32_t*)(tri + (size_t)(nt + 1) * 3);
    uint8_t* alive = S->alive.as<uint8_t>();
    uint32_t* misc = S->misc.as<uint32_t>();
    uint8_t* ever = nullptr;
    for (int a = 0; a < 3; a++) S->corner[a] = corner[a];
    if (nv && nt && (edge_crossings || march_mesh) && coherent) {
        if ((rc = S->ever.grow(ctx, 2 * (size_t)nv + 64))) return rc;
        ever = S->ever.as<uint8_t>();
        CX_HIP(ctx, hipMemsetAsync(ever, 0, nv, st));
    }
    if (nv && nt) {
        hipLaunchKernelGGL(cxp_k_tri_prio, dim3(cx_blocks(nt)), dim3(256), 0, st, tri, prio, nt, tprio3);
        cxp_weld_params W;
        for (int a = 0; a < 3; a++) W.ex[a] = std::trunc((10000 * 1.0) / corner[a]);
        W.thr = 0.0;
        if (edge_crossings && !cx_debug_knob("CX_WELD_ALL", 0)) {
            const double exmin = std::min(W.ex[0], std::min(W.ex[1], W.ex[2]));
            if (exmin >= 16.0) W.thr = 2.0 / exmin + 1e-9;
        }
        const u64 wsz = W.thr > 0.0 ? cxp_edge_table_size(nv) : cx_table_size(nv);
        if ((rc = S->tkeys.grow(ctx, std::max(wsz, cx_table_size(nt)) * sizeof(u64)))) return rc;
        if ((rc = S->tvals.grow(ctx, wsz * sizeof(u64)))) return rc;
        hipLaunchKernelGGL(cxp_k_fill64, dim3(2048), dim3(256), 0, st, S->tkeys.as<u64>(), (size_t)wsz, CXD_EMPTY);
        hipLaunchKernelGGL(cxp_k_fill64, dim3(2048), dim3(256), 0, st, S->tvals.as<u64>(), (size_t)wsz, (u64)0);
        hipLaunchKernelGGL(cxp_k_weld_insert, dim3(cx_blocks(nv)), dim3(256), 0, st, pts, prio, nv, W, S->tkeys.as<u64>(), S->tvals.as<u64>(), wsz - 1, vkeep);
        hipLaunchKernelGGL(cxp_k_weld_lookup, dim3(cx_blocks(nv)), dim3(256), 0, st, pts, nv, W, S->tkeys.as<u64>(), S->tvals.as<u64>(), wsz - 1, rep, vkeep, prio);
        uint8_t* involved = (coherent && !cx_debug_knob("CX_DEDUPE_ALL", 0)) ? moved : nullptr;
        if (involved) CX_HIP(ctx, hipMemsetAsync(involved, 0, nv, st));
        hipLaunchKernelGGL(cxp_k_remap, dim3(cx_blocks(nt)), dim3(256), 0, st, tri, alive, nt, rep, (const u64*)nullptr, involved, ever);
        const u64 tsz = involved ? cxp_edge_table_size(nt) : cx_table_size(nt);
        hipLaunchKernelGGL(cxp_k_fill64, dim3(2048), dim3(256), 0, st, S->tkeys.as<u64>(), (size_t)tsz, CXD_EMPTY);
        hipLaunchKernelGGL(cxp_k_dedupe_insert, dim3(cx_blocks(nt)), dim3(256), 0, st, tri, tprio3, alive, nt, S->tkeys.as<u64>(), tsz - 1, (const uint8_t*)involved);
        hipLaunchKernelGGL(cxp_k_dedupe_resolve, dim3(cx_blocks(nt)), dim3(256), 0, st, tri, alive, nt, S->tkeys.as<u64>(), tsz - 1, (const uint8_t*)involved);
        CX_HIP(ctx, hipMemsetAsync(misc + 4, 0, 2 * sizeof(uint32_t), st));
        hipLaunchKernelGGL(cxp_k_count_alive, dim3(std::min(cx_blocks(nt), 1024u)), dim3(256), 0, st, alive, nt, misc + 4);
        if (smooth > 0.0) {
            const u64 esz = cx_table_size((size_t)nt * 3);
            if ((rc = S->tkeys.grow(ctx, esz * sizeof(u64)))) return rc;
            if ((rc = S->pts_out.grow(ctx, (size_t)(nv + 1) * 3 * sizeof(double)))) return rc;
            if ((rc = S->flags.grow(ctx, (size_t)(nv + nt + 16) * sizeof(uint32_t)))) return rc;
            double* sum = S->pts_out.as<double>();
            uint32_t* cnt = S->flags.as<uint32_t>();
            CX_HIP(ctx, hipMemsetAsync(sum, 0, (size_t)nv * 3 * sizeof(double), st));
            CX_HIP(ctx, hipMemsetAsync(cnt, 0, (size_t)nv * sizeof(uint32_t), st));
            hipLaunchKernelGGL(cxp_k_fill64, dim3(2048), dim3(256), 0, st, S->tkeys.as<u64>(), (size_t)esz, CXD_EMPTY);
            if (cx_debug_knob("CX_SMOOTH_TWO_STEP", 0)) {
                hipLaunchKernelGGL(cxp_k_unique_edges, dim3(cx_blocks(nt)), dim3(256), 0, st, tri, alive, nt, S->tkeys.as<u64>(), esz - 1);
                hipLaunchKernelGGL(cxp_k_smooth_accumulate, dim3(cx_blocks(esz)), dim3(256), 0, st, S->tkeys.as<const u64>(), (size_t)esz, pts, sum, cnt);
            } else {
                hipLaunchKernelGGL(cxp_k_smooth_edges, dim3(cx_blocks(nt)), dim3(256), 0, st, tri, alive, nt, S->tkeys.as<u64>(), esz - 1, (const double*)pts, sum, cnt);
            }
            hipLaunchKernelGGL(cxp_k_smooth_apply, dim3(cx_blocks(nv)), dim3(256), 0, st, pts, sum, cnt, nv, smooth);
        }
        u64* parent = S->parent.as<u64>();
        hipLaunchKernelGGL(cxp_k_iota64, dim3(cx_blocks(nv)), dim3(256), 0, st, parent, nv);
        CX_HIP(ctx, hipMemsetAsync(moved, 0, nv, st));
        hipLaunchKernelGGL(cxp_k_tiny, dim3(cx_blocks(nt)), dim3(256), 0, st, tri, alive, nt, pts, 1.0 / corner[0], 1.0 / corner[1],
                           1.0 / corner[2], 1e-4, parent, prio, moved);
        hipLaunchKernelGGL(cxp_k_move, dim3(cx_blocks(nv)), dim3(256), 0, st, pts, pts, parent, moved, nv);
        hipLaunchKernelGGL(cxp_k_count_alive, dim3(std::min(cx_blocks(nt), 1024u)), dim3(256), 0, st, alive, nt, misc + 5);
        uint32_t h[2];
        CX_HIP(ctx, hipMemcpyAsync(h, misc + 4, 2 * sizeof(uint32_t), hipMemcpyDeviceToHost, st));
        CX_HIP(ctx, hipStreamSynchronize(st));
        counts[2] = h[0]; counts[3] = h[1];
    }
    return cxp_clean_orient(ctx, S, nv, nt, do_clean, true, tprio3, counts, coherent,
                            (coherent && nv && nt && !cx_debug_knob("CX_DEDUPE_ALL", 0)) ? moved : nullptr, shard, ever);
}

extern "C" int cx_postprocess3d_ex(cx_ctx* ctx, uint32_t flags, double smooth, int64_t* out_counts) {
    if (!ctx) return CX_ERR_INVALID;
    if (!ctx->extracted) { ctx->err = "cx_postprocess3d: no valid extraction"; return CX_ERR_STATE; }
    CX_HIP(ctx, hipSetDevice(ctx->device));
    cx_post_state* S;
    int rc = cxp_state(ctx, &S);
    if (rc) return rc;
    const uint32_t nv = (uint32_t)ctx->counts.n_vertices, nt = (uint32_t)ctx->counts.n_triangles;
    hipStream_t st = ctx->stream;
    int64_t counts[8] = {0, 0, 0, 0, 0, 0, 0, 0};
    if ((rc = cxp_reserve3d(ctx, S, nv, nt))) return rc;
    const cx_params& P = ctx->last;
    const uint8_t* vkeep = nullptr;
    cxp_origin3 org{{0.0, 0.0, 0.0}};
    if (ctx->origin[0] < 0 || ctx->origin[1] < 0 || ctx->origin[2] < 0)
        for (int a = 0; a < 3; a++) org.o[a] = (double)ctx->origin[a];
    if (nv && nt) {
        cxp_launch_vertices_f64(dim3(cx_blocks(nv)), st, P.grid, ctx->grid64_valid ? ctx->grid64.get() : nullptr, P.n1, P.n2,
                           P.div_plane, P.div_row, P.value, ctx->verts.get(), nv, S->pts.as<double>(), S->prio.as<uint32_t>(), org);
        CX_HIP(ctx, hipMemcpyAsync(S->tri.get(), ctx->tris, (size_t)nt * 3 * sizeof(int32_t), hipMemcpyDeviceToDevice, st));
        if (ctx->keep_valid) {
            CX_HIP(ctx, hipMemcpyAsync(S->alive.get(), ctx->tri_keep, nt, hipMemcpyDeviceToDevice, st));
            vkeep = ctx->tri_keep + nt;
        } else {
            CX_HIP(ctx, hipMemsetAsync(S->alive.get(), 1, nt, st));
        }
    }
    double corner[3] = {(double)(P.n0 - 1), (double)(P.n1 - 1), (double)(P.n2 - 1)};
    for (int a = 0; a < 3; a++)
        if (ctx->corner_ref[a] > 0) corner[a] = (double)ctx->corner_ref[a];
    if ((rc = cxp_run3d(ctx, S, nv, nt, corner, vkeep, !(flags & 1u), smooth, true, counts, true))) return rc;
    ctx->post_valid = true;
    S->keys_edge = true;
    if (out_counts) memcpy(out_counts, counts, sizeof(counts));
    return CX_OK;
}

extern "C" int cx_postprocess3d_capped(cx_ctx* ctx, uint32_t flags, int64_t* out_counts) {
    if (!ctx) return CX_ERR_INVALID;
    if (!ctx->extracted) { ctx->err = "cx_postprocess3d_capped: no valid extraction"; return CX_ERR_STATE; }
    if (flags & ~1u) { ctx->err = "cx_postprocess3d_capped: unknown flag bits (only bit 0, no clean-up, is defined)"; return CX_ERR_INVALID; }
    CX_HIP(ctx, hipSetDevice(ctx->device));
    cx_cap_view K;
    int rc = cx_cap_view_get(ctx, "cx_postprocess3d_capped", &K);
    if (rc) return rc;
    cx_post_state* S;
    if ((rc = cxp_state(ctx, &S))) return rc;
    const uint32_t nv0 = (uint32_t)ctx->counts.n_vertices, nt0 = (uint32_t)ctx->counts.n_triangles;
    const uint32_t nv = nv0 + K.ncv, nt = nt0 + K.nct;
    hipStream_t st = ctx->stream;
    int64_t counts[8] = {0, 0, 0, 0, 0, 0, 0, 0};
    if ((rc = cxp_reserve3d(ctx, S, nv, nt))) return rc;
    const cx_params& P = ctx->last;
    const cxp_origin3 org{{0.0, 0.0, 0.0}};
    if (nv && nt) {
        const double* A64 = ctx->grid64_valid ? ctx->grid64.get() : nullptr;
        if (nv0) cxp_launch_vertices_f64(dim3(cx_blocks(nv0)), st, P.grid, A64, P.n1, P.n2, P.div_plane, P.div_row, P.value, (const cx_vrec*)ctx->verts.get(), nv0,
                                         S->pts.as<double>(), S->prio.as<uint32_t>(), org);
        if (K.ncv) cxp_launch_vertices_f64(dim3(cx_blocks(K.ncv)), st, P.grid, A64, P.n1, P.n2, P.div_plane, P.div_row, P.value, K.vrec, K.ncv,
                                           S->pts.as<double>() + (size_t)nv0 * 3, S->prio.as<uint32_t>() + nv0, org);
        if (nt0) CX_HIP(ctx, hipMemcpyAsync(S->tri.get(), ctx->tris, (size_t)nt0 * 3 * sizeof(int32_t), hipMemcpyDeviceToDevice, st));
        if (K.nct) CX_HIP(ctx, hipMemcpyAsync(S->tri.as<int32_t>() + (size_t)nt0 * 3, K.tris, (size_t)K.nct * 3 * sizeof(int32_t), hipMemcpyDeviceToDevice, st));
        CX_HIP(ctx, hipMemsetAsync(S->alive.get(), 1, nt, st));
    }
    const double corner[3] = {(double)(P.n0 - 1), (double)(P.n1 - 1), (double)(P.n2 - 1)};
    if ((rc = cxp_run3d(ctx, S, nv, nt, corner, nullptr, !(flags & 1u), 0.0, true, counts, true))) return rc;
    ctx->post_valid = true;
    S->keys_edge = true;
    S->capped_gen = S->gen;
    if (out_counts) memcpy(out_counts, counts, sizeof(counts));
    return CX_OK;
}
bool cx_level1_capped(cx_ctx* ctx) { return ctx->post && ctx->post_valid && ctx->post->capped(); }

extern "C" int cx_postprocess3d_shard_begin(cx_ctx* ctx, uint32_t flags, int64_t own_lo, int64_t own_hi, int64_t* out_counts,
                                            int64_t* n_own_lower, int64_t* n_upper_copies, int64_t* n_candidates) {
    if (!ctx || !n_own_lower || !n_upper_copies || !n_candidates) return CX_ERR_INVALID;
    if (!ctx->extracted) { ctx->err = "cx_postprocess3d_shard_begin: no valid extraction"; return CX_ERR_STATE; }
    const cx_params& P = ctx->last;
    if (own_lo < 0 || own_hi <= own_lo || own_hi > (int64_t)P.n0 - 1) { ctx->err = "cx_postprocess3d_shard_begin: own cell layers outside the local array"; return CX_ERR_INVALID; }
    if (ctx->keep_valid) { ctx->err = "cx_postprocess3d_shard_begin: not after a seeded selection"; return CX_ERR_STATE; }
    if (ctx->origin[0] < 0) { ctx->err = "cx_postprocess3d_shard_begin: the local array starts before the volume (cx_set_origin)"; return CX_ERR_STATE; }
    CX_HIP(ctx, hipSetDevice(ctx->device));
    cx_post_state* S;
    int rc = cxp_state(ctx, &S);
    if (rc) return rc;
    const uint32_t nv = (uint32_t)ctx->counts.n_vertices, nt = (uint32_t)ctx->counts.n_triangles;
    hipStream_t st = ctx->stream;
    int64_t counts[8] = {0, 0, 0, 0, 0, 0, 0, 0};
    if ((rc = cxp_reserve3d(ctx, S, nv, nt))) return rc;
    const cxp_origin3 org{{(double)ctx->origin[0], (double)ctx->origin[1], (double)ctx->origin[2]}};
    if (nv && nt) {
        cxp_launch_vertices_f64(dim3(cx_blocks(nv)), st, P.grid, ctx->grid64_valid ? ctx->grid64.get() : nullptr, P.n1, P.n2,
                           P.div_plane, P.div_row, P.value, ctx->verts.get(), nv, S->pts.as<double>(), S->prio.as<uint32_t>(), org);
        CX_HIP(ctx, hipMemcpyAsync(S->tri.get(), ctx->tris, (size_t)nt * 3 * sizeof(int32_t), hipMemcpyDeviceToDevice, st));
        CX_HIP(ctx, hipMemsetAsync(S->alive.get(), 1, nt, st));
    }
    double corner[3] = {(double)(P.n0 - 1), (double)(P.n1 - 1), (double)(P.n2 - 1)};
    for (int a = 0; a < 3; a++)
        if (ctx->corner_ref[a] > 0) corner[a] = (double)ctx->corner_ref[a];
    const cxp_shard sh{P.n1 * P.n2, (uint32_t)own_lo, (uint32_t)own_hi, P.n0 - 1};
    ctx->post_valid = false;
    if ((rc = cxp_run3d(ctx, S, nv, nt, corner, nullptr, !(flags & 1u), 0.0, true, counts, true, &sh))) return rc;
    if (out_counts) memcpy(out_counts, counts, sizeof(counts));
    *n_own_lower = S->shard.n1;
    *n_upper_copies = S->shard.n4;
    *n_candidates = S->shard.ncand;
    return CX_OK;
}

extern "C" int cx_postprocess3d_shard_boundary(cx_ctx* ctx, int which, uint64_t* hash, uint32_t* label) {
    if (!ctx || (which != 1 && which != 4)) return CX_ERR_INVALID;
    if (!ctx->post || !ctx->post->shard.open) { ctx->err = "cx_postprocess3d_shard_boundary: call cx_postprocess3d_shard_begin first"; return CX_ERR_STATE; }
    CX_HIP(ctx, hipSetDevice(ctx->device));
    cx_post_state* S = ctx->post;
    const size_t n1 = S->shard.n1, n4 = S->shard.n4, nb = n1 + n4;
    const size_t n = which == 1 ? n1 : n4;
    if (!n) return CX_OK;
    if (!hash || !label) return CX_ERR_INVALID;
    const u64* hash1 = S->bnd.as<const u64>();
    const cxp_cand* cand = (const cxp_cand*)(hash1 + nb);
    const uint32_t* label1 = (const uint32_t*)(cand + nb);
    CX_HIP(ctx, hipMemcpyAsync(hash, which == 1 ? hash1 : hash1 + n1, n * sizeof(u64), hipMemcpyDefault, ctx->stream));
    CX_HIP(ctx, hipMemcpyAsync(label, which == 1 ? label1 : label1 + n1, n * sizeof(uint32_t), hipMemcpyDefault, ctx->stream));
    CX_HIP(ctx, hipStreamSynchronize(ctx->stream));
    return CX_OK;
}

extern "C" int cx_postprocess3d_shard_candidates(cx_ctx* ctx, uint32_t* cand_label, double* cand_x, uint32_t* cand_vertex_key, double* cand_nx,
                                                 uint8_t* cand_negative, uint8_t* cand_has) {
    if (!ctx) return CX_ERR_INVALID;
    if (!ctx->post || !ctx->post->shard.open) { ctx->err = "cx_postprocess3d_shard_candidates: call cx_postprocess3d_shard_begin first"; return CX_ERR_STATE; }
    CX_HIP(ctx, hipSetDevice(ctx->device));
    cx_post_state* S = ctx->post;
    const size_t nb = (size_t)S->shard.n1 + S->shard.n4, nc = S->shard.ncand;
    if (!nc) return CX_OK;
    if (!cand_label || !cand_x || !cand_vertex_key || !cand_nx || !cand_negative || !cand_has) return CX_ERR_INVALID;
    const cxp_cand* cand = (const cxp_cand*)(S->bnd.as<const u64>() + nb);
    std::vector<cxp_cand> h(nc);
    CX_HIP(ctx, hipMemcpyAsync(h.data(), cand, nc * sizeof(cxp_cand), hipMemcpyDeviceToHost, ctx->stream));
    CX_HIP(ctx, hipStreamSynchronize(ctx->stream));
    for (size_t i = 0; i < nc; i++) {
        cand_label[i] = h[i].label; cand_x[i] = h[i].x; cand_vertex_key[i] = h[i].vkey; cand_nx[i] = h[i].nx;
        cand_negative[i] = (uint8_t)h[i].sign; cand_has[i] = (uint8_t)h[i].has;
    }
    return CX_OK;
}

extern "C" int cx_postprocess3d_shard_finish(cx_ctx* ctx, const uint32_t* labels, const uint8_t* flips, int64_t n, int64_t* out_counts) {
    if (!ctx || n < 0 || (n && (!labels || !flips))) return CX_ERR_INVALID;
    if (!ctx->post || !ctx->post->shard.open) { ctx->err = "cx_postprocess3d_shard_finish: call cx_postprocess3d_shard_begin first"; return CX_ERR_STATE; }
    if (n > (int64_t)ctx->post->shard.nt2) { ctx->err = "cx_postprocess3d_shard_finish: more labels than triangles"; return CX_ERR_INVALID; }
    CX_HIP(ctx, hipSetDevice(ctx->device));
    int64_t counts[8] = {0, 0, 0, 0, 0, 0, 0, 0};
    int rc = cxp_shard_finish(ctx, ctx->post, labels, flips, (uint32_t)n, counts);
    if (rc) return rc;
    ctx->post_valid = true;
    if (out_counts) memcpy(out_counts, counts, sizeof(counts));
    return CX_OK;
}

extern "C" int cx_level1_download_keys(cx_ctx* ctx, uint32_t* keys) {
    if (!ctx || !keys) return CX_ERR_INVALID;
    if (!ctx->post || !ctx->post_valid || !ctx->post->keys_valid) { ctx->err = "cx_level1_download_keys: run cx_postprocess3d first"; return CX_ERR_STATE; }
    CX_HIP(ctx, hipSetDevice(ctx->device));
    cx_post_state* S = ctx->post;
    if (!S->nv_out) return CX_OK;
    return cx_copy_to_host1(ctx, keys, S->keys_out.get(), (size_t)S->nv_out * sizeof(uint32_t));
}

extern "C" int cx_level0_points_f64(cx_ctx* ctx, double* points_xyz) {
    if (!ctx || !points_xyz) return CX_ERR_INVALID;
    if (!ctx->extracted) { ctx->err = "cx_level0_points_f64: no valid extraction"; return CX_ERR_STATE; }
    CX_HIP(ctx, hipSetDevice(ctx->device));
    cx_post_state* S;
    int rc = cxp_state(ctx, &S);
    if (rc) return rc;
    const uint32_t nv = (uint32_t)ctx->counts.n_vertices;
    if (!nv) return CX_OK;
    if ((rc = S->pts.grow(ctx, (size_t)(nv + 1) * 3 * sizeof(double)))) return rc;
    if ((rc = S->prio.grow(ctx, (size_t)(nv + 1) * sizeof(uint32_t)))) return rc;
    const cx_params& P = ctx->last;
    const cxp_origin3 org{{(double)ctx->origin[0], (double)ctx->origin[1], (double)ctx->origin[2]}};
    cxp_launch_vertices_f64(dim3(cx_blocks(nv)), ctx->stream, P.grid, ctx->grid64_valid ? ctx->grid64.get() : nullptr, P.n1, P.n2,
                       P.div_plane, P.div_row, P.value, ctx->verts.get(), nv, S->pts.as<double>(), S->prio.as<uint32_t>(), org);
    if ((rc = cx_copy_to_host1(ctx, points_xyz, S->pts.get(), (size_t)nv * 3 * sizeof(double)))) return rc;
    ctx->post_valid = false;
    return CX_OK;
}

extern "C" int cx_postprocess3d_mesh(cx_ctx* ctx, const double* points_xyz, int64_t nv64, const int32_t* tris, int64_t nt64, const int64_t* corner3,
                                     uint32_t flags, double smooth, int64_t* out_counts) {
    if (!ctx || !corner3 || nv64 < 0 || nt64 < 0 || (nv64 && !points_xyz) || (nt64 && !tris)) return CX_ERR_INVALID;
    if (nv64 >= 0x7FFFFFFFLL || nt64 >= 0x7FFFFFFFLL || corner3[0] < 1 || corner3[1] < 1 || corner3[2] < 1) {
        ctx->err = "cx_postprocess3d_mesh: corner >= 1 per axis and fewer than 2^31 vertices / triangles";
        return CX_ERR_INVALID;
    }
    CX_HIP(ctx, hipSetDevice(ctx->device));
    cx_post_state* S;
    int rc = cxp_state(ctx, &S);
    if (rc) return rc;
    const uint32_t nv = (uint32_t)nv64, nt = (uint32_t)nt64;
    {
        int32_t lo = 0, hi = -1;
        for (int64_t n = 0; n < nt64 * 3; n++) { lo = tris[n] < lo ? tris[n] : lo; hi = tris[n] > hi ? tris[n] : hi; }
        if (lo < 0 || (int64_t)hi >= nv64) { ctx->err = "cx_postprocess3d_mesh: triangle index out of range"; return CX_ERR_INVALID; }
    }
    hipStream_t st = ctx->stream;
    int64_t counts[8] = {0, 0, 0, 0, 0, 0, 0, 0};
    if ((rc = cxp_reserve3d(ctx, S, nv, nt))) return rc;
    if (nv && nt) {
        CX_HIP(ctx, hipMemcpyAsync(S->pts.get(), points_xyz, (size_t)nv * 3 * sizeof(double), hipMemcpyHostToDevice, st));
        CX_HIP(ctx, hipMemcpyAsync(S->tri.get(), tris, (size_t)nt * 3 * sizeof(int32_t), hipMemcpyHostToDevice, st));
        CX_HIP(ctx, hipMemsetAsync(S->alive.get(), 1, nt, st));
        hipLaunchKernelGGL(cxp_k_iota_prio, dim3(cx_blocks(nv)), dim3(256), 0, st, S->prio.as<uint32_t>(), nv);
    }
    const double corner[3] = {(double)corner3[0], (double)corner3[1], (double)corner3[2]};
    if ((rc = cxp_run3d(ctx, S, nv, nt, corner, nullptr, !(flags & 1u), smooth, !(flags & 4u), counts, false, nullptr, (flags & 8u) != 0u))) return rc;
    ctx->post_valid = true;
    if (out_counts) memcpy(out_counts, counts, sizeof(counts));
    return CX_OK;
}

extern "C" int cx_level1_download(cx_ctx* ctx, double* points_xyz, int32_t* tris) {
    if (!ctx) return CX_ERR_INVALID;
    if (!ctx->post || !ctx->post_valid) { ctx->err = "cx_level1_download: run cx_postprocess3d first"; return CX_ERR_STATE; }
    CX_HIP(ctx, hipSetDevice(ctx->device));
    cx_post_state* S = ctx->post;
    void* d[2] = {(points_xyz && S->nv_out) ? (void*)points_xyz : nullptr, (tris && S->nt_out) ? (void*)tris : nullptr};
    const void* sp[2] = {S->pts_out.get(), S->tri_out.get()};
    const size_t nb[2] = {(size_t)S->nv_out * 3 * sizeof(double), (size_t)S->nt_out * 3 * sizeof(int32_t)};
    return cx_copy_to_host(ctx, 2, d, sp, nb);
}

extern "C" int cx_level1_device_ptrs(cx_ctx* ctx, void** points_xyz, void** tris, int64_t* n_vertices, int64_t* n_triangles) {
    if (!ctx) return CX_ERR_INVALID;
    if (!ctx->post || !ctx->post_valid) { ctx->err = "cx_level1_device_ptrs: run cx_postprocess3d first"; return CX_ERR_STATE; }
    CX_HIP(ctx, hipSetDevice(ctx->device));
    CX_HIP(ctx, hipStreamSynchronize(ctx->stream));
    cx_post_state* S = ctx->post;
    if (points_xyz) *points_xyz = S->nv_out ? S->pts_out.get() : nullptr;
    if (tris) *tris = S->nt_out ? S->tri_out.get() : nullptr;
    if (n_vertices) *n_vertices = (int64_t)S->nv_out;
    if (n_triangles) *n_triangles = (int64_t)S->nt_out;
    return CX_OK;
}

__global__ void cxp_k_vertex_flip(const int32_t* __restrict__ tri, uint32_t nt, const u64* __restrict__ parent, const u64* __restrict__ cflip,
                                  uint8_t* __restrict__ vflip) {
    const uint32_t t = blockIdx.x * blockDim.x + threadIdx.x;
    if (t >= nt) return;
    const uint8_t f = (uint8_t)(cflip[(uint32_t)parent[t]] & 1u);
    if (!f) return;
#pragma unroll
    for (int k = 0; k < 3; k++) vflip[(uint32_t)tri[(size_t)t * 3 + k]] = 1;
}
int cx_level1_attr_view(cx_ctx* ctx, const char* who, cx_level1_view* out) {
    if (!ctx->post || !ctx->post_valid || !ctx->post->keys_valid) { ctx->err = std::string(who) + ": no Level-1 mesh (run cx_postprocess3d first)"; return CX_ERR_INVALID; }
    cx_post_state* S = ctx->post;
    if (!S->keys_edge) {
        ctx->err = std::string(who) + (S->clipped ? ": the vertices of a clipped mesh (cx_level1_clip_*) are not all edge crossings of the resident array"
                                       : S->simplified ? ": the vertices of a simplified mesh (cx_level1_simplify) are cluster means, not edge crossings of the resident array"
                                                     : ": the Level-1 vertices are not edge crossings of the resident array (a mesh handed to cx_postprocess3d_mesh, or a shard)");
        return CX_ERR_UNSUPPORTED;
    }
    const uint32_t nv = (uint32_t)S->nv_out, nt = (uint32_t)S->nt_out;
    if (nv && !S->vflip_valid) {
        if (nt && (!S->orient_live || S->orient_nt != nt)) { ctx->err = std::string(who) + ": the orientation tables of the post-pass are gone (run cx_postprocess3d again)"; return CX_ERR_STATE; }
        int rc;
        if ((rc = S->vflip.grow(ctx, (size_t)nv + 16))) return rc;
        CX_HIP(ctx, hipMemsetAsync(S->vflip.get(), 0, nv, ctx->stream));
        if (nt) {
            const u64* parent = S->parent.as<const u64>();
            const u64* cflip = S->comp.as<const u64>() + nt;
            hipLaunchKernelGGL(cxp_k_vertex_flip, dim3(cx_blocks(nt)), dim3(256), 0, ctx->stream, S->tri_out.as<const int32_t>(), nt, parent, cflip, S->vflip.as<uint8_t>());
            CX_HIP(ctx, hipGetLastError());
        }
        S->vflip_valid = true;
    }
    out->keys = S->keys_out.as<const uint32_t>();
    out->vflip = S->vflip.as<const uint8_t>();
    out->nv = nv;
    return CX_OK;
}

__global__ void cxp_k_carry_normals(const double* __restrict__ in, const uint32_t* __restrict__ use, const uint32_t* __restrict__ vnew, uint32_t n,
                                    double* __restrict__ out) {
    const uint32_t v = blockIdx.x * blockDim.x + threadIdx.x;
    if (v >= n || (use && !use[v])) return;
    const uint32_t j = vnew[v];
    if (j == 0xFFFFFFFFu) return;
#pragma unroll
    for (int a = 0; a < 3; a++) out[(size_t)j * 3 + a] = in[(size_t)v * 3 + a];
}
int cx_level1_comp_view_get(cx_ctx* ctx, const char* who, cx_level1_comp_view* out) {
    if (!ctx->post || !ctx->post_valid || !ctx->post->keys_valid) { ctx->err = std::string(who) + ": no Level-1 mesh (run cx_postprocess3d first)"; return CX_ERR_INVALID; }
    cx_post_state* S = ctx->post;
    if (S->shard_mesh || S->shard.open) {
        ctx->err = std::string(who) + ": the components of a sharded Level-1 mesh reach other ranks (cx_postprocess3d_shard_*): not available";
        return CX_ERR_UNSUPPORTED;
    }
    const uint32_t nv = (uint32_t)S->nv_out, nt = (uint32_t)S->nt_out;
    if ((nt && (!S->orient_live || S->orient_nt != nt)) || (!nt && S->orient_nt && !S->orient_live)) {
        ctx->err = std::string(who) + ": the orientation tables of the post-pass are gone (a 4-D pass used their memory, or the post-pass ran without the orientation step): run cx_postprocess3d again";
        return CX_ERR_STATE;
    }
    out->parent = S->parent.as<const u64>();
    out->cflip = nt ? S->comp.as<const u64>() + nt : nullptr;
    out->tri = S->tri_out.as<const int32_t>();
    out->pts = S->pts_out.as<const double>();
    out->keys = S->keys_out.as<const uint32_t>();
    out->nv = nv; out->nt = nt;
    for (int a = 0; a < 3; a++) out->corner[a] = S->corner[a];
    out->gen = S->gen;
    return CX_OK;
}
int cx_level1_comp_scratch_get(cx_ctx* ctx, cx_level1_comp_scratch* out) {
    cx_post_state* S = ctx->post;
    const size_t nv = (size_t)S->nv_out, nt = (size_t)S->nt_out;
    int rc;
    if ((rc = S->pts.grow(ctx, (nv + 1) * 3 * sizeof(double)))) return rc;
    if ((rc = S->tri.grow(ctx, (nt + 1) * 3 * sizeof(int32_t)))) return rc;
    if ((rc = S->keys_tmp.grow(ctx, (nv + 1) * sizeof(uint32_t)))) return rc;
    if ((rc = S->tkeys.grow(ctx, (nt + 1) * 2 * sizeof(u64)))) return rc;
    out->pts = S->pts.as<double>();
    out->tri = S->tri.as<int32_t>();
    out->keys = S->keys_tmp.as<uint32_t>();
    out->parent = S->tkeys.as<u64>();
    out->cflip = out->parent + nt + 1;
    return CX_OK;
}
int cx_level1_comp_commit(cx_ctx* ctx, uint32_t nv_new, uint32_t nt_new, const uint32_t* vuse, const uint32_t* vnew) {
    cx_post_state* S = ctx->post;
    hipStream_t st = ctx->stream;
    S->smap_valid = false;
    if (S->carried && nv_new && S->nv_out) {
        const int rcn = S->nrm[1 - S->nrm_cur].grow(ctx, ((size_t)nv_new + 1) * 3 * sizeof(double));
        if (rcn) return rcn;
        hipLaunchKernelGGL(cxp_k_carry_normals, dim3(cx_blocks((size_t)S->nv_out)), dim3(256), 0, st, S->nrm[S->nrm_cur].as<const double>(), vuse, vnew,
                           (uint32_t)S->nv_out, S->nrm[1 - S->nrm_cur].as<double>());
        S->nrm_cur = 1 - S->nrm_cur;
    }
    const size_t nt_old = (size_t)S->nt_out;
    const u64* parent_new = S->tkeys.as<const u64>();
    if (nv_new) {
        CX_HIP(ctx, hipMemcpyAsync(S->pts_out.get(), S->pts.get(), (size_t)nv_new * 3 * sizeof(double), hipMemcpyDeviceToDevice, st));
        CX_HIP(ctx, hipMemcpyAsync(S->keys_out.get(), S->keys_tmp.get(), (size_t)nv_new * sizeof(uint32_t), hipMemcpyDeviceToDevice, st));
    }
    if (nt_new) {
        CX_HIP(ctx, hipMemcpyAsync(S->tri_out.get(), S->tri.get(), (size_t)nt_new * 3 * sizeof(int32_t), hipMemcpyDeviceToDevice, st));
        CX_HIP(ctx, hipMemcpyAsync(S->parent.get(), parent_new, (size_t)nt_new * sizeof(u64), hipMemcpyDeviceToDevice, st));
        CX_HIP(ctx, hipMemcpyAsync(S->comp.as<u64>() + nt_new, parent_new + nt_old + 1, (size_t)nt_new * sizeof(u64), hipMemcpyDeviceToDevice, st));
    }
    CX_HIP(ctx, hipStreamSynchronize(st));
    S->nv_out = nv_new; S->nt_out = nt_new;
    S->orient_nt = nt_new;
    S->vflip_valid = false;
    const bool capped = S->capped();
    S->gen++;
    if (capped) S->capped_gen = S->gen;
    return CX_OK;
}

int cx_level1_simplify_bufs(cx_ctx* ctx, bool normals, bool dry_run, cx_level1_simplify_io* out) {
    cx_post_state* S = ctx->post;
    const size_t nv = (size_t)S->nv_out, nt = (size_t)S->nt_out;
    int rc;
    if ((rc = S->pts.grow(ctx, (nv + 1) * 3 * sizeof(double)))) return rc;
    if ((rc = S->prio.grow(ctx, (nv + 1) * sizeof(uint32_t)))) return rc;
    if ((rc = S->tri.grow(ctx, (nt + 1) * 3 * sizeof(int32_t) * 2))) return rc;
    if ((rc = S->alive.grow(ctx, nt + 16))) return rc;
    if ((rc = S->parent2.grow(ctx, (nv + 1) * sizeof(u64)))) return rc;
    if ((rc = (dry_run ? S->rep : S->smap).grow(ctx, (nv + 16) * sizeof(int32_t)))) return rc;
    if (normals && (rc = S->nrm_tmp.grow(ctx, (nv + 1) * 3 * sizeof(double)))) return rc;
    out->pts = S->pts.as<double>();
    out->prio = S->prio.as<uint32_t>();
    out->tri = S->tri.as<int32_t>();
    out->tprio3 = (uint32_t*)(out->tri + (nt + 1) * 3);
    out->alive = S->alive.as<uint8_t>();
    out->map = (dry_run ? S->rep : S->smap).as<int32_t>();
    out->nrm_new = normals ? S->nrm_tmp.as<double>() : nullptr;
    out->nrm_src = S->carried ? S->nrm[S->nrm_cur].as<const double>() : nullptr;
    out->simplified = S->simplified;
    if (!dry_run) S->smap_valid = false;
    return CX_OK;
}
__global__ void cxp_k_simplify_map(int32_t* map, uint32_t nv_old, uint32_t ncl, const u64* parent2, const uint32_t* vnew) {
    const uint32_t v = blockIdx.x * blockDim.x + threadIdx.x;
    if (v >= nv_old) return;
    int32_t c = map[v];
    if (c < 0 || (uint32_t)c >= ncl) { map[v] = -1; return; }
    if (parent2) { uint32_t par; c = (int32_t)cxp_find(parent2, (uint32_t)c, par); }
    map[v] = (int32_t)vnew[c];
}
int cx_level1_simplify_tail(cx_ctx* ctx, uint32_t nv_old, uint32_t ncl, uint32_t nt, bool do_clean, bool normals, int64_t* counts) {
    cx_post_state* S = ctx->post;
    hipStream_t st = ctx->stream;
    int rc;
    int32_t* tri = S->tri.as<int32_t>();
    uint32_t* tprio3 = (uint32_t*)(tri + ((size_t)S->nt_out + 1) * 3);
    uint8_t* alive = S->alive.as<uint8_t>();
    const int cur = S->nrm_cur;
    if (nt && ncl) {
        const u64 tsz = cx_table_size(nt);
        if ((rc = S->tkeys.grow(ctx, tsz * sizeof(u64)))) return rc;
        hipLaunchKernelGGL(cxp_k_fill64, dim3(2048), dim3(256), 0, st, S->tkeys.as<u64>(), (size_t)tsz, CXD_EMPTY);
        hipLaunchKernelGGL(cxp_k_dedupe_insert, dim3(cx_blocks(nt)), dim3(256), 0, st, tri, tprio3, alive, nt, S->tkeys.as<u64>(), tsz - 1, (const uint8_t*)nullptr);
        hipLaunchKernelGGL(cxp_k_dedupe_resolve, dim3(cx_blocks(nt)), dim3(256), 0, st, tri, alive, nt, S->tkeys.as<u64>(), tsz - 1, (const uint8_t*)nullptr);
    }
    if ((rc = S->scan.grow(ctx, ((size_t)ncl + 16) * sizeof(uint32_t)))) return rc;
    if (ncl) CX_HIP(ctx, hipMemsetAsync(S->scan.get(), 0xFF, (size_t)ncl * sizeof(uint32_t), st));
    if (normals && (rc = S->nrm[1 - cur].grow(ctx, ((size_t)ncl + 1) * 3 * sizeof(double)))) return rc;
    if ((rc = cxp_clean_orient(ctx, S, ncl, nt, do_clean, true, tprio3, counts, true))) { ctx->post_valid = false; return rc; }
    const uint32_t* vnew = S->scan.as<const uint32_t>();
    if (nv_old) hipLaunchKernelGGL(cxp_k_simplify_map, dim3(cx_blocks(nv_old)), dim3(256), 0, st, S->smap.as<int32_t>(), nv_old, ncl,
                                   (do_clean && nt) ? S->parent2.as<const u64>() : (const u64*)nullptr, vnew);
    if (normals && ncl && S->nv_out) {
        hipLaunchKernelGGL(cxp_k_carry_normals, dim3(cx_blocks(ncl)), dim3(256), 0, st, S->nrm_tmp.as<const double>(), (const uint32_t*)nullptr, vnew, ncl,
                           S->nrm[1 - cur].as<double>());
        S->nrm_cur = 1 - cur;
    }
    CX_HIP(ctx, hipGetLastError());
    CX_HIP(ctx, hipStreamSynchronize(st));
    S->simplified = true; S->carried = normals;
    S->smap_valid = true; S->smap_n = nv_old;
    return CX_OK;
}
int cx_level1_carried_normals(cx_ctx* ctx, const double** nrm, uint32_t* nv) {
    cx_post_state* S = ctx->post;
    if (!S || !ctx->post_valid || !S->keys_valid || !S->simplified) return 0;
    *nv = (uint32_t)S->nv_out;
    *nrm = S->carried ? S->nrm[S->nrm_cur].as<const double>() : nullptr;
    return S->carried ? 1 : 2;
}
int cx_level1_simplify_map_get(cx_ctx* ctx, const int32_t** map, uint32_t* n) {
    cx_post_state* S = ctx->post;
    if (!S || !ctx->post_valid || !S->simplified || !S->smap_valid) {
        ctx->err = "cx_level1_simplify_map: no simplification since the last post-pass or filter";
        return CX_ERR_STATE;
    }
    *map = S->smap.as<const int32_t>(); *n = S->smap_n;
    return CX_OK;
}

int cx_level1_clip_bufs(cx_ctx* ctx, size_t nv_raw, size_t nt_raw, cx_level1_clip_io* out) {
    cx_post_state* S = ctx->post;
    int rc;
    if ((rc = S->pts.grow(ctx, (nv_raw + 1) * 3 * sizeof(double)))) return rc;
    if ((rc = S->prio.grow(ctx, (nv_raw + 1) * sizeof(uint32_t)))) return rc;
    if ((rc = S->tri.grow(ctx, (nt_raw + 1) * 3 * sizeof(int32_t) * 2))) return rc;
    if ((rc = S->alive.grow(ctx, nt_raw + 16))) return rc;
    if ((rc = S->parent2.grow(ctx, (nv_raw + 1) * sizeof(u64)))) return rc;
    out->pts = S->pts.as<double>();
    out->prio = S->prio.as<uint32_t>();
    out->tri = S->tri.as<int32_t>();
    out->tprio3 = (uint32_t*)(out->tri + (nt_raw + 1) * 3);
    out->alive = S->alive.as<uint8_t>();
    return CX_OK;
}
int cx_level1_clip_tail(cx_ctx* ctx, uint32_t nv_raw, uint32_t nt_raw, bool do_clean, int64_t* counts) {
    cx_post_state* S = ctx->post;
    int rc;
    uint32_t* tprio3 = (uint32_t*)(S->tri.as<int32_t>() + ((size_t)nt_raw + 1) * 3);
    if ((rc = cxp_clean_orient(ctx, S, nv_raw, nt_raw, do_clean, true, tprio3, counts, true))) { ctx->post_valid = false; return rc; }
    CX_HIP(ctx, hipStreamSynchronize(ctx->stream));
    S->simplified = true; S->carried = false; S->clipped = true;
    return CX_OK;
}
int cx_level1_clip_normals(cx_ctx* ctx, double** out) {
    cx_post_state* S = ctx->post;
    const int cur = S->nrm_cur;
    const int rc = S->nrm[1 - cur].grow(ctx, ((size_t)S->nv_out + 1) * 3 * sizeof(double));
    if (rc) return rc;
    *out = S->nrm[1 - cur].as<double>();
    S->nrm_cur = 1 - cur;
    S->carried = true;
    return CX_OK;
}
uint64_t cx_level1_generation(cx_ctx* ctx) {
    cx_post_state* S = ctx->post;
    return (S && ctx->post_valid && S->keys_valid) ? S->gen : 0;
}

extern "C" int cx_surface_geometry(cx_ctx* ctx, double* points_xyz, int64_t* nv_io, int32_t* tris, int64_t* nt_io, int mode) {
    if (!ctx || !points_xyz || !tris || !nv_io || !nt_io || mode < 0 || mode > 2) return CX_ERR_INVALID;
    if (*nv_io < 0 || *nt_io < 0 || *nv_io > 0x7FFFFFF0LL || *nt_io > 0x7FFFFFF0LL) return CX_ERR_INVALID;
    CX_HIP(ctx, hipSetDevice(ctx->device));
    cx_post_state* S;
    int rc = cxp_state(ctx, &S);
    if (rc) return rc;
    const uint32_t nv = (uint32_t)*nv_io, nt = (uint32_t)*nt_io;
    for (int64_t n = 0; n < (int64_t)nt * 3; n++)
        if (tris[n] < 0 || tris[n] >= (int64_t)nv) { ctx->err = "cx_surface_geometry: triangle index out of range"; return CX_ERR_INVALID; }
    hipStream_t st = ctx->stream;
    if ((rc = S->pts.grow(ctx, (size_t)(nv + 1) * 3 * sizeof(double)))) return rc;
    if ((rc = S->prio.grow(ctx, (size_t)(nv + 1) * sizeof(uint32_t)))) return rc;
    if ((rc = S->tri.grow(ctx, (size_t)(nt + 1) * 3 * sizeof(int32_t) * 2))) return rc;
    if ((rc = S->alive.grow(ctx, (size_t)nt + 16))) return rc;
    if ((rc = S->parent2.grow(ctx, (size_t)(nv + 1) * sizeof(u64)))) return rc;
    int32_t* tri = S->tri.as<int32_t>();
    uint32_t* tprio3 = (uint32_t*)(tri + (size_t)(nt + 1) * 3);
    if (nv) CX_HIP(ctx, hipMemcpyAsync(S->pts.get(), points_xyz, (size_t)nv * 3 * sizeof(double), hipMemcpyHostToDevice, st));
    if (nt) CX_HIP(ctx, hipMemcpyAsync(tri, tris, (size_t)nt * 3 * sizeof(int32_t), hipMemcpyHostToDevice, st));
    if (nv) hipLaunchKernelGGL(cxp_k_iota_prio, dim3(cx_blocks(nv)), dim3(256), 0, st, S->prio.as<uint32_t>(), nv);
    if (nt) {
        CX_HIP(ctx, hipMemsetAsync(S->alive.get(), 1, nt, st));
        hipLaunchKernelGGL(cxp_k_tri_prio, dim3(cx_blocks(nt)), dim3(256), 0, st, tri, S->prio.as<const uint32_t>(), nt, tprio3);
        hipLaunchKernelGGL(cxp_k_remap, dim3(cx_blocks(nt)), dim3(256), 0, st, tri, S->alive.as<uint8_t>(), nt, S->prio.as<const uint32_t>(),
                           (const u64*)nullptr);
    }
    int64_t counts[8] = {0, 0, 0, 0, 0, 0, 0, 0};
    if ((rc = cxp_clean_orient(ctx, S, nv, nt, mode != 0, mode != 2, tprio3, counts, false))) return rc;
    if (S->nv_out) CX_HIP(ctx, hipMemcpyAsync(points_xyz, S->pts_out.get(), (size_t)S->nv_out * 3 * sizeof(double), hipMemcpyDeviceToHost, st));
    if (S->nt_out) CX_HIP(ctx, hipMemcpyAsync(tris, S->tri_out.get(), (size_t)S->nt_out * 3 * sizeof(int32_t), hipMemcpyDeviceToHost, st));
    CX_HIP(ctx, hipStreamSynchronize(st));
    *nv_io = S->nv_out; *nt_io = S->nt_out;
    ctx->post_valid = false;
    return CX_OK;
}
```

Measured before the change: 456,500.

## Fold init passes into existing kernels and drop host syncs in postprocess

Replaces the iterative host-synchronised union-find flatten loop with an in-kernel path-compressing find inside comp_maxx. Folds iota, memset and triangle-priority initialisation into the weld_lookup, remap, move and edges_claim kernels. Merges the two me_count launches into one, vectorises count_alive, and defers count readbacks through pinned host words and events. Adds a bounded-probe first edge table that retries at full size when it overflows. This cuts kernel launches, memsets and host round-trips at the cost of more complex, state-dependent initialisation ordering.

```diff
diff --git a/contourist_amd/csrc/cx_post.h b/contourist_amd/csrc/cx_post.h
--- a/contourist_amd/csrc/cx_post.h
+++ b/contourist_amd/csrc/cx_post.h
@@ -40,6 +40,8 @@
     std::vector<int64_t> me_off;
     int64_t nv_out = 0, nt_out = 0;
     int64_t ms_out = 0, mt_out = 0;
+    uint32_t* hwords = nullptr;
+    hipEvent_t hev[2] = {nullptr, nullptr};
 };
 
 int cxp_state(cx_ctx* ctx, cx_post_state** out);
@@ -53,7 +55,7 @@
 int cxp_scan(cx_ctx* ctx, cx_post_state* S, const uint32_t* in, uint32_t* out, uint32_t n, uint32_t* total_dev);
 
 int cxp_orient_pick(cx_ctx* ctx, const int32_t* tri, uint32_t nt, const double* pts, u64* parent, u64* comp, const uint32_t* keys,
-                    const uint8_t* cls, uint32_t* clist, uint32_t* misc);
+                    const uint8_t* cls, uint32_t* clist, uint32_t* misc, bool misc_cleared = false);
 int cxp_orient_decide(cx_ctx* ctx, int32_t* tri, uint32_t nt, const double* pts, const u64* parent, u64* comp, const uint32_t* clist,
                       uint32_t* misc, bool wind, uint32_t* ncomp);
 
diff --git a/contourist_amd/csrc/cx_post.hip b/contourist_amd/csrc/cx_post.hip
--- a/contourist_amd/csrc/cx_post.hip
+++ b/contourist_amd/csrc/cx_post.hip
@@ -1,5 +1,6 @@
 #include <algorithm>
 #include <cmath>
+#include <cstdio>
 #include <cstring>
 #include <new>
 #include <string>
@@ -11,6 +12,9 @@
     if (!ctx->post) return;
     cx_post_state* S = ctx->post;
     if (S->me_pinned) (void)hipHostFree(S->me_pinned);
+    if (S->hwords) (void)hipHostFree(S->hwords);
+    for (hipEvent_t e : S->hev)
+        if (e) (void)hipEventDestroy(e);
     delete S;
     ctx->post = nullptr;
 }
@@ -22,26 +26,22 @@
 __global__ void cxp_k_fill64(u64* a, size_t n, u64 v) {
     for (size_t i = blockIdx.x * (size_t)blockDim.x + threadIdx.x; i < n; i += (size_t)gridDim.x * blockDim.x) a[i] = v;
 }
-__global__ void cxp_k_jump(u64* parent, uint32_t n, uint32_t* changed) {
-    const uint32_t i = blockIdx.x * blockDim.x + threadIdx.x;
-    if (i >= n) return;
-    u64 w = parent[i];
+__device__ __forceinline__ uint32_t cxp_flatten_one(u64* parent, uint32_t i) {
+    const u64 w = __hip_atomic_load(&parent[i], __ATOMIC_RELAXED, __HIP_MEMORY_SCOPE_AGENT);
     uint32_t p = (uint32_t)w;
-    if (p == i) return;
+    if (p == i) return i;
+    uint32_t par = (uint32_t)(w >> 32) & 1u;
     bool moved = false;
-#pragma unroll 1
-    for (int hop = 0; hop < 3; hop++) {
-        const u64 wp = parent[p];
+    for (;;) {
+        const u64 wp = __hip_atomic_load(&parent[p], __ATOMIC_RELAXED, __HIP_MEMORY_SCOPE_AGENT);
         const uint32_t pp = (uint32_t)wp;
         if (pp == p) break;
-        w = ((((w >> 32) ^ (wp >> 32)) & 1ULL) << 32) | (u64)pp;
+        par ^= (uint32_t)(wp >> 32) & 1u;
         p = pp;
         moved = true;
     }
-    if (moved) {
-        parent[i] = w;
-        *changed = 1u;
-    }
+    if (moved) __hip_atomic_store(&parent[i], ((u64)par << 32) | (u64)p, __ATOMIC_RELAXED, __HIP_MEMORY_SCOPE_AGENT);
+    return p;
 }
 
 #define CXP_SCAN_BLOCK 1024u
@@ -198,39 +198,18 @@
     atomicMax(&tvals[slot], ((u64)prio[v] << 32) | (u64)v);
 }
 __global__ void cxp_k_weld_lookup(const double* pts, uint32_t nv, cxp_weld_params W, const u64* tkeys, const u64* tvals, u64 mask,
-                                  uint32_t* rep, const uint8_t* vkeep, const uint32_t* prio) {
+                                  uint32_t* rep, const uint8_t* vkeep, const uint32_t* prio, u64* parent, uint8_t* involved, uint8_t* ever) {
     const uint32_t v = blockIdx.x * blockDim.x + threadIdx.x;
     if (v >= nv) return;
+    parent[v] = (u64)v;
+    if (involved) involved[v] = 0;
+    if (ever) ever[v] = 0;
     if (vkeep && !vkeep[v]) { rep[v] = v; return; }
     if (cxp_weld_alone(pts + (size_t)v * 3, prio[v], W)) { rep[v] = v; return; }
     const u64 key = cxp_weld_key(pts + (size_t)v * 3, W);
     u64 slot = cxd_mix(key) & mask;
     while (tkeys[slot] != key) slot = (slot + 1) & mask;
     rep[v] = (uint32_t)tvals[slot];
-}
-
-__global__ void cxp_k_remap(int32_t* tri, uint8_t* alive, uint32_t nt, const uint32_t* map, const u64* parent, uint8_t* involved = nullptr,
-                            uint8_t* ever = nullptr) {
-    const uint32_t t = blockIdx.x * blockDim.x + threadIdx.x;
-    if (t >= nt || !alive[t]) return;
-    const uint32_t x[3] = {(uint32_t)tri[(size_t)t * 3], (uint32_t)tri[(size_t)t * 3 + 1], (uint32_t)tri[(size_t)t * 3 + 2]};
-    uint32_t v[3];
-    if (map) {
-        v[0] = map[x[0]]; v[1] = map[x[1]]; v[2] = map[x[2]];
-    } else {
-        uint32_t par;
-#pragma unroll
-        for (int s = 0; s < 3; s++) v[s] = cxp_find(parent, x[s], par);
-    }
-#pragma unroll
-    for (int s = 0; s < 3; s++) {
-        if (v[s] != x[s]) {
-            tri[(size_t)t * 3 + s] = (int32_t)v[s];
-            if (involved) involved[v[s]] = 1;
-            if (ever) ever[v[s]] = 1;
-        }
-    }
-    if (v[0] == v[1] || v[0] == v[2] || v[1] == v[2]) alive[t] = 0;
 }
 
 struct cxp_tri3 {
@@ -247,6 +226,34 @@
     if (p.a != q.a) return p.a < q.a;
     if (p.b != q.b) return p.b < q.b;
     return p.c < q.c;
+}
+
+__global__ void cxp_k_remap(int32_t* tri, uint8_t* alive, uint32_t nt, const uint32_t* map, const u64* parent, uint8_t* involved = nullptr,
+                            uint8_t* ever = nullptr, const uint32_t* prio = nullptr, uint32_t* tprio3 = nullptr) {
+    const uint32_t t = blockIdx.x * blockDim.x + threadIdx.x;
+    if (t >= nt || !alive[t]) return;
+    const uint32_t x[3] = {(uint32_t)tri[(size_t)t * 3], (uint32_t)tri[(size_t)t * 3 + 1], (uint32_t)tri[(size_t)t * 3 + 2]};
+    uint32_t v[3];
+    if (map) {
+        v[0] = map[x[0]]; v[1] = map[x[1]]; v[2] = map[x[2]];
+        if (tprio3) {
+            const cxp_tri3 p = cxp_sorted3(prio[x[0]], prio[x[1]], prio[x[2]]);
+            tprio3[(size_t)t * 3] = p.a; tprio3[(size_t)t * 3 + 1] = p.b; tprio3[(size_t)t * 3 + 2] = p.c;
+        }
+    } else {
+        uint32_t par;
+#pragma unroll
+        for (int s = 0; s < 3; s++) v[s] = cxp_find(parent, x[s], par);
+    }
+#pragma unroll
+    for (int s = 0; s < 3; s++) {
+        if (v[s] != x[s]) {
+            tri[(size_t)t * 3 + s] = (int32_t)v[s];
+            if (involved) involved[v[s]] = 1;
+            if (ever) ever[v[s]] = 1;
+        }
+    }
+    if (v[0] == v[1] || v[0] == v[2] || v[1] == v[2]) alive[t] = 0;
 }
 
 __global__ void cxp_k_dedupe_insert(const int32_t* tri, const uint32_t* tprio3, const uint8_t* alive, uint32_t nt, u64* table,
@@ -300,7 +307,19 @@
     if (threadIdx.x == 0) s_n = 0;
     __syncthreads();
     uint32_t n = 0;
-    for (uint32_t t = blockIdx.x * blockDim.x + threadIdx.x; t < nt; t += gridDim.x * blockDim.x) n += alive[t] ? 1u : 0u;
+    const uint32_t nq = nt / 16u;
+    for (uint32_t q = blockIdx.x * blockDim.x + threadIdx.x; q < nq; q += gridDim.x * blockDim.x) {
+        const uint4 w = reinterpret_cast<const uint4*>(alive)[q];
+        const uint32_t x[4] = {w.x, w.y, w.z, w.w};
+#pragma unroll
+        for (int k = 0; k < 4; k++) {
+            uint32_t b = x[k] | (x[k] >> 4);
+            b |= b >> 2;
+            b |= b >> 1;
+            n += __popc(b & 0x01010101u);
+        }
+    }
+    if (blockIdx.x == 0 && threadIdx.x < nt - nq * 16u) n += alive[nq * 16u + threadIdx.x] ? 1u : 0u;
 #pragma unroll
     for (int o = 32; o > 0; o >>= 1) n += (uint32_t)__shfl_xor((int)n, o);
     if ((threadIdx.x & 63u) == 0 && n) atomicAdd(&s_n, n);
@@ -328,9 +347,13 @@
         moved[v0] = moved[v1] = moved[v2] = 1;
     }
 }
-__global__ void cxp_k_move(double* pts, const double* pts_src, const u64* parent, const uint8_t* moved, uint32_t nv) {
+__global__ void cxp_k_move(double* pts, const double* pts_src, const u64* parent, uint8_t* moved, uint32_t nv, u64* next, uint8_t* used) {
     const uint32_t v = blockIdx.x * blockDim.x + threadIdx.x;
-    if (v >= nv || !moved[v]) return;
+    if (v >= nv) return;
+    if (next) next[v] = (u64)v;
+    if (used) used[v] = 0;
+    if (!moved[v]) return;
+    moved[v] = 0;
     uint32_t par;
     const uint32_t r = cxp_find(parent, v, par);
 #pragma unroll
@@ -380,11 +403,16 @@
     block_total = s[255];
     return s[threadIdx.x] - t;
 }
-__global__ __launch_bounds__(256) void cxp_k_me_count(const uint8_t* flags, uint32_t n, uint32_t* count) {
+__global__ __launch_bounds__(256) void cxp_k_me_count2(const uint8_t* flags_a, uint32_t na, uint32_t* count_a, uint32_t nba, const uint8_t* flags_b, uint32_t nb,
+                                                       uint32_t* count_b) {
     __shared__ uint32_t s_n;
     if (threadIdx.x == 0) s_n = 0;
     __syncthreads();
-    const uint32_t base = blockIdx.x * CXP_SCAN_BLOCK + threadIdx.x * 4u;
+    const bool first = blockIdx.x < nba;
+    const uint8_t* flags = first ? flags_a : flags_b;
+    const uint32_t n = first ? na : nb, block = first ? blockIdx.x : blockIdx.x - nba;
+    uint32_t* count = first ? count_a : count_b;
+    const uint32_t base = block * CXP_SCAN_BLOCK + threadIdx.x * 4u;
     uint32_t c = 0;
     if (base + 3u < n) {
         const uint32_t w = *reinterpret_cast<const uint32_t*>(flags + base);
@@ -396,7 +424,7 @@
     for (int o = 32; o > 0; o >>= 1) c += (uint32_t)__shfl_xor((int)c, o);
     if ((threadIdx.x & 63u) == 0 && c) atomicAdd(&s_n, c);
     __syncthreads();
-    if (threadIdx.x == 0) count[blockIdx.x] = s_n;
+    if (threadIdx.x == 0) count[block] = s_n;
 }
 __global__ void cxp_k_mark_used8(const int32_t* tri, const uint8_t* alive, uint32_t nt, uint8_t* used) {
     const uint32_t t = blockIdx.x * blockDim.x + threadIdx.x;
@@ -454,9 +482,10 @@
     const uint32_t a = tri[(size_t)t * 3], b = tri[(size_t)t * 3 + 1], c = tri[(size_t)t * 3 + 2];
     return ((a == lo && b == hi) || (b == lo && c == hi) || (c == lo && a == hi)) ? 1u : 0u;
 }
-__global__ void cxp_k_edges_claim(const int32_t* tri, uint32_t nt, u64* tab, u64 mask, u64 mult) {
+__global__ void cxp_k_edges_claim(const int32_t* tri, uint32_t nt, u64* tab, u64 mask, u64 mult, u64* parent) {
     const uint32_t t = blockIdx.x * blockDim.x + threadIdx.x;
     if (t >= nt) return;
+    parent[t] = (u64)t;
     const uint32_t v[3] = {(uint32_t)tri[(size_t)t * 3], (uint32_t)tri[(size_t)t * 3 + 1], (uint32_t)tri[(size_t)t * 3 + 2]};
     for (int e = 0; e < 3; e++) {
         const uint32_t p = v[e], q = v[(e + 1) % 3];
@@ -654,11 +683,11 @@
     }
     for (uint32_t x = threadIdx.x; x < CXP_EB; x += 256u) {
         if (b0 + x >= nt) continue;
-        const uint32_t r = cxp_lfind(lp, x);
-        if (r != x) parent[b0 + x] = (u64)(b0 + r);
-    }
-}
-__global__ void cxp_k_edges_link_far(const int32_t* tri, uint32_t nt, const u64* tab, u64 mask, u64 mult, const uint8_t* others, u64* parent) {
+        parent[b0 + x] = (u64)(b0 + cxp_lfind(lp, x));
+    }
+}
+__global__ void cxp_k_edges_link_far(const int32_t* tri, uint32_t nt, const u64* tab, u64 mask, u64 mult, const uint8_t* others, u64* parent,
+                                     uint32_t probe_limit) {
     const uint32_t t = blockIdx.x * blockDim.x + threadIdx.x;
     if (t >= nt) return;
     const uint32_t fb = others[t];
@@ -671,20 +700,35 @@
         const uint32_t lo = min(p, q), hi = max(p, q);
         const u64 key = ((u64)lo << 32) | (u64)hi;
         u64 slot = cxp_edge_slot(lo, hi, mask, mult);
-        while (tab[2 * slot] != key) slot = (slot + 1) & mask;
+        uint32_t probes = 0;
+        while (tab[2 * slot] != key && probes < probe_limit) { slot = (slot + 1) & mask; probes++; }
+        if (probes >= probe_limit) continue;
         const uint32_t o = (uint32_t)tab[2 * slot + 1];
         if (o != t) cxp_union0(parent, t, o);
     }
 }
+__global__ __launch_bounds__(256) void cxp_k_count_keys(const u64* tab, size_t slots, uint32_t* counter) {
+    uint32_t n = 0;
+    for (size_t i = blockIdx.x * (size_t)blockDim.x + threadIdx.x; i < slots; i += (size_t)gridDim.x * blockDim.x) n += tab[2 * i] != CXD_EMPTY ? 1u : 0u;
+    n = cxd_wave_add(n);
+    if ((threadIdx.x & 63u) == 0 && n) atomicAdd(counter, n);
+}
 #define CXP_OWN(cls, t) (!(cls) || (cls)[t] <= 2u)
-__global__ void cxp_k_comp_maxx(const int32_t* tri, uint32_t nt, const double* pts, const u64* parent, u64* cmaxx, const uint8_t* cls) {
+__global__ void cxp_k_comp_maxx(const int32_t* tri, uint32_t nt, const double* pts, u64* parent, u64* cmaxx, const uint8_t* cls) {
     const uint32_t idx = blockIdx.x * blockDim.x + threadIdx.x;
     const uint32_t t = nt - 1u - idx;
     const bool have = idx < nt && CXP_OWN(cls, t);
     uint32_t root = 0;
     u64 m = 0;
+    if (idx < nt) {
+        root = cxp_flatten_one(parent, t);
+        if (root == t) {
+            cmaxx[(size_t)nt + t] = 0;
+            cmaxx[2 * (size_t)nt + t] = 0;
+            ((uint32_t*)(cmaxx + 3 * (size_t)nt))[t] = 0u;
+        }
+    }
     if (have) {
-        root = (uint32_t)parent[t];
 #pragma unroll
         for (int s = 0; s < 3; s++) m = max(m, cxd_orderable(pts[(size_t)tri[(size_t)t * 3 + s] * 3]));
     }
@@ -888,34 +932,28 @@
     return CX_OK;
 }
 
-static int cxp_flatten(cx_ctx* ctx, u64* parent, uint32_t n, uint32_t* changed_dev) {
-    for (int it = 0; it < 64; it++) {
-        CX_HIP(ctx, hipMemsetAsync(changed_dev, 0, sizeof(uint32_t), ctx->stream));
-        hipLaunchKernelGGL(cxp_k_jump, dim3(cx_blocks(n)), dim3(256), 0, ctx->stream, parent, n, changed_dev);
-        uint32_t changed = 0;
-        CX_HIP(ctx, hipMemcpyAsync(&changed, changed_dev, sizeof(uint32_t), hipMemcpyDeviceToHost, ctx->stream));
-        CX_HIP(ctx, hipStreamSynchronize(ctx->stream));
-        if (!changed) return CX_OK;
-    }
-    ctx->err = "union-find did not flatten";
-    return CX_ERR_HIP;
+static int cxp_host_words(cx_ctx* ctx, cx_post_state* S) {
+    if (!S->hwords) CX_HIP(ctx, hipHostMalloc((void**)&S->hwords, 16 * sizeof(uint32_t), hipHostMallocDefault));
+    for (hipEvent_t& e : S->hev)
+        if (!e) CX_HIP(ctx, hipEventCreateWithFlags(&e, hipEventDisableTiming));
+    return CX_OK;
 }
 
 int cxp_orient_pick(cx_ctx* ctx, const int32_t* tri, uint32_t nt, const double* pts, u64* parent, u64* comp, const uint32_t* keys,
-                    const uint8_t* cls, uint32_t* clist, uint32_t* misc) {
-    int rc;
+                    const uint8_t* cls, uint32_t* clist, uint32_t* misc, bool misc_cleared) {
     hipStream_t st = ctx->stream;
     u64* cmaxx = comp;
     u64* cbest = cmaxx + nt;
     u64* cmaxv = cbest + nt;
     uint32_t* cstart = (uint32_t*)(cmaxv + nt);
-    if ((rc = cxp_flatten(ctx, parent, nt, misc))) return rc;
-    CX_HIP(ctx, hipMemsetAsync(cmaxx, 0, (size_t)nt * (3 * sizeof(u64) + sizeof(uint32_t)), st));
-    CX_HIP(ctx, hipMemsetAsync(misc + 3, 0, sizeof(uint32_t), st));
+    CX_HIP(ctx, hipMemsetAsync(cmaxx, 0, (size_t)nt * sizeof(u64), st));
+    if (!misc_cleared) {
+        CX_HIP(ctx, hipMemsetAsync(misc + 3, 0, sizeof(uint32_t), st));
+        CX_HIP(ctx, hipMemsetAsync(misc + 11, 0, sizeof(uint32_t), st));
+    }
     hipLaunchKernelGGL(cxp_k_comp_maxx, dim3(cx_blocks(nt)), dim3(256), 0, st, tri, nt, pts, parent, cmaxx, cls);
     const uint32_t* cn = misc + 11;
     const dim3 lgrid(std::min(cx_blocks(nt), 1024u));
-    CX_HIP(ctx, hipMemsetAsync(misc + 11, 0, sizeof(uint32_t), st));
     hipLaunchKernelGGL(cxp_k_comp_list, dim3(cx_blocks(nt)), dim3(256), 0, st, tri, nt, pts, parent, cmaxx, cls, clist, misc + 11);
     hipLaunchKernelGGL(cxp_k_comp_maxv, lgrid, dim3(256), 0, st, tri, nt, pts, parent, cmaxx, cmaxv, keys, cls, (const uint32_t*)clist, cn);
     hipLaunchKernelGGL(cxp_k_comp_start, lgrid, dim3(256), 0, st, tri, nt, pts, parent, cmaxv, cbest, cls, (const uint32_t*)clist, cn);
@@ -939,8 +977,11 @@
 
 static int cxp_clean_orient(cx_ctx* ctx, cx_post_state* S, uint32_t nv, uint32_t nt, bool do_clean, bool do_orient,
                             uint32_t* tprio3, int64_t* out_counts, bool coherent, uint8_t* involved = nullptr, const cxp_shard* shard = nullptr,
-                            uint8_t* ever = nullptr) {
+                            uint8_t* ever = nullptr,
+                            bool prepared = false) {
     int rc;
+    const bool parent2_set = prepared, counts_pending = prepared;
+    if ((rc = cxp_host_words(ctx, S))) return rc;
     double* pts = S->pts.as<double>();
     uint32_t* prio = S->prio.as<uint32_t>();
     int32_t* tri = S->tri.as<int32_t>();
@@ -952,11 +993,12 @@
     S->shard_mesh = false; S->gen++; S->orient_nt = 0;
     S->shard.open = false;
     S->simplified = false; S->carried = false; S->smap_valid = false; S->clipped = false;
+    if (!prepared) CX_HIP(ctx, hipMemsetAsync(misc + 3, 0, 11 * sizeof(uint32_t), st));
     if (do_clean && nt) {
         u64* parent2 = S->parent2.as<u64>();
-        hipLaunchKernelGGL(cxp_k_iota64, dim3(cx_blocks(nv)), dim3(256), 0, st, parent2, nv);
+        if (!parent2_set) hipLaunchKernelGGL(cxp_k_iota64, dim3(cx_blocks(nv)), dim3(256), 0, st, parent2, nv);
         hipLaunchKernelGGL(cxp_k_degenerate, dim3(cx_blocks(nt)), dim3(256), 0, st, tri, alive, nt, pts, parent2, prio);
-        if (involved) CX_HIP(ctx, hipMemsetAsync(involved, 0, nv, st));
+        if (involved && !prepared) CX_HIP(ctx, hipMemsetAsync(involved, 0, nv, st));
         hipLaunchKernelGGL(cxp_k_remap, dim3(cx_blocks(nt)), dim3(256), 0, st, tri, alive, nt, (const uint32_t*)nullptr, parent2, involved, ever);
         const u64 tsz = involved ? cxp_edge_table_size(nt) : cx_table_size(nt);
         if ((rc = S->tkeys.grow(ctx, tsz * sizeof(u64)))) return rc;
@@ -971,7 +1013,6 @@
         if ((rc = S->told.grow(ctx, ((size_t)nt + 16) * sizeof(uint32_t)))) return rc;
         cls = S->cls.as<uint8_t>();
         told = S->told.as<uint32_t>();
-        CX_HIP(ctx, hipMemsetAsync(misc + 6, 0, 2 * sizeof(uint32_t), st));
         if (nt) hipLaunchKernelGGL(cxp_k_shard_classify, dim3(cx_blocks(nt)), dim3(256), 0, st, tprio3, alive, nt, *shard, cx_fdiv_make(shard->plane), cls, misc + 6);
     }
     if ((rc = S->flags.grow(ctx, (size_t)(nv + nt + 16) * sizeof(uint32_t)))) return rc;
@@ -984,27 +1025,27 @@
     uint32_t* toff = voff + nbv + 8;
     uint32_t nv2 = 0, nt2 = 0;
     if (nt) {
-        CX_HIP(ctx, hipMemsetAsync(used, 0, (size_t)nv, st));
+        if (!prepared) CX_HIP(ctx, hipMemsetAsync(used, 0, (size_t)nv, st));
         hipLaunchKernelGGL(cxp_k_mark_used8, dim3(cx_blocks(nt)), dim3(256), 0, st, tri, alive, nt, used);
-        hipLaunchKernelGGL(cxp_k_me_count, dim3(nbv), dim3(256), 0, st, (const uint8_t*)used, nv, voff);
-        hipLaunchKernelGGL(cxp_k_me_count, dim3(nbt), dim3(256), 0, st, (const uint8_t*)alive, nt, toff);
+        hipLaunchKernelGGL(cxp_k_me_count2, dim3(nbv + nbt), dim3(256), 0, st, (const uint8_t*)used, nv, voff, nbv, (const uint8_t*)alive, nt, toff);
         hipLaunchKernelGGL(cxp_k_scan_sums2, dim3(2), dim3(1024), 0, st, voff, nbv, misc + 1, toff, nbt, misc + 2);
-        uint32_t h[2];
-        CX_HIP(ctx, hipMemcpyAsync(h, misc + 1, 2 * sizeof(uint32_t), hipMemcpyDeviceToHost, st));
-        CX_HIP(ctx, hipStreamSynchronize(st));
-        nv2 = h[0]; nt2 = h[1];
-    }
-    if ((rc = S->pts_out.grow(ctx, (size_t)(nv2 + 1) * 3 * sizeof(double)))) return rc;
-    if ((rc = S->tri_out.grow(ctx, (size_t)(nt2 + 1) * 3 * sizeof(int32_t)))) return rc;
-    if ((rc = S->keys_out.grow(ctx, (size_t)(nv2 + 1) * sizeof(uint32_t)))) return rc;
+        CX_HIP(ctx, hipMemcpyAsync(S->hwords + 1, misc + 1, 5 * sizeof(uint32_t), hipMemcpyDeviceToHost, st));
+        CX_HIP(ctx, hipEventRecord(S->hev[0], st));
+    }
+    if ((rc = S->pts_out.grow(ctx, (size_t)(nv + 1) * 3 * sizeof(double)))) return rc;
+    if ((rc = S->tri_out.grow(ctx, (size_t)(nt + 1) * 3 * sizeof(int32_t)))) return rc;
+    if ((rc = S->keys_out.grow(ctx, (size_t)(nv + 1) * sizeof(uint32_t)))) return rc;
     double* pts2 = S->pts_out.as<double>();
     int32_t* tri2 = S->tri_out.as<int32_t>();
     uint32_t* keys2 = S->keys_out.as<uint32_t>();
-    if (nt2) {
-        hipLaunchKernelGGL(cxp_k_compact_pts_fused, dim3(nbv), dim3(256), 0, st, (const double*)pts, (const uint8_t*)used, (const uint32_t*)voff, nv, vnew, pts2,
-                           (const uint32_t*)prio, keys2, (const uint8_t*)ever, ever ? ever + nv : nullptr);
+    if (nt) {
+        if (nbv) hipLaunchKernelGGL(cxp_k_compact_pts_fused, dim3(nbv), dim3(256), 0, st, (const double*)pts, (const uint8_t*)used, (const uint32_t*)voff, nv, vnew, pts2,
+                                    (const uint32_t*)prio, keys2, (const uint8_t*)ever, ever ? ever + nv : nullptr);
         hipLaunchKernelGGL(cxp_k_compact_tri_fused, dim3(nbt), dim3(256), 0, st, (const int32_t*)tri, (const uint8_t*)alive, (const uint32_t*)toff,
                            (const uint32_t*)vnew, nt, tri2, told);
+        CX_HIP(ctx, hipEventSynchronize(S->hev[0]));
+        nv2 = S->hwords[1]; nt2 = S->hwords[2];
+        if (counts_pending && out_counts) { out_counts[2] = S->hwords[4]; out_counts[3] = S->hwords[5]; }
     }
     S->nv_out = nv2; S->nt_out = nt2;
     S->keys_valid = true;
@@ -1032,25 +1073,31 @@
         u64* cmaxv = cbest + nt2;
         uint32_t* cstart = (uint32_t*)(cmaxv + nt2);
         uint32_t* others = S->comp.as<uint32_t>();
-        for (;;) {
+        uint32_t* clist = S->flags.as<uint32_t>();
+        const bool count_entries = blocks && cx_debug_knob("CX_EDGE_TABLE_COUNT", 0);
+        for (bool repeat = false;; repeat = true) {
+            if (repeat) {
+                CX_HIP(ctx, hipMemsetAsync(misc + 3, 0, sizeof(uint32_t), st));
+                CX_HIP(ctx, hipMemsetAsync(misc + 11, 0, 3 * sizeof(uint32_t), st));
+            }
             if ((rc = S->tkeys.grow(ctx, 2 * esz * sizeof(u64)))) return rc;
             u64* etab = S->tkeys.as<u64>();
             hipLaunchKernelGGL(cxp_k_fill64, dim3(2048), dim3(256), 0, st, etab, (size_t)(2 * esz), CXD_EMPTY);
-            hipLaunchKernelGGL(cxp_k_iota64, dim3(cx_blocks(nt2)), dim3(256), 0, st, parent, nt2);
-            const u64 emult = (blocks && esz != esz_full) ? 0 : std::max<u64>(1, esz / std::max<u64>(1, (u64)nv2));
+            const bool first_table = blocks && esz != esz_full;
+            const u64 emult = first_table ? 0 : std::max<u64>(1, esz / std::max<u64>(1, (u64)nv2));
             if (blocks) {
-                CX_HIP(ctx, hipMemsetAsync(misc + 12, 0, sizeof(uint32_t), st));
+                const uint32_t probe_limit = first_table ? 256u : 0xFFFFFFFFu;
                 hipLaunchKernelGGL(cxp_k_edges_block, dim3((nt2 + CXP_EB - 1u) / CXP_EB), dim3(256), 0, st, tri2, nt2, (const uint8_t*)(ever + nv), etab, esz - 1,
-                                   emult, parent, (uint8_t*)others, esz == esz_full ? 0xFFFFFFFFu : 256u, misc + 12);
-                if (esz != esz_full) {
-                    uint32_t over = 0;
-                    CX_HIP(ctx, hipMemcpyAsync(&over, misc + 12, sizeof(uint32_t), hipMemcpyDeviceToHost, st));
-                    CX_HIP(ctx, hipStreamSynchronize(st));
-                    if (over) { esz = esz_full; continue; }
+                                   emult, parent, (uint8_t*)others, probe_limit, misc + 12);
+                if (first_table) {
+                    if (count_entries) hipLaunchKernelGGL(cxp_k_count_keys, dim3(1024), dim3(256), 0, st, (const u64*)etab, (size_t)esz, misc + 13);
+                    CX_HIP(ctx, hipMemcpyAsync(S->hwords + 12, misc + 12, 2 * sizeof(uint32_t), hipMemcpyDeviceToHost, st));
+                    CX_HIP(ctx, hipEventRecord(S->hev[1], st));
                 }
-                hipLaunchKernelGGL(cxp_k_edges_link_far, dim3(cx_blocks(nt2)), dim3(256), 0, st, tri2, nt2, etab, esz - 1, emult, (const uint8_t*)others, parent);
+                hipLaunchKernelGGL(cxp_k_edges_link_far, dim3(cx_blocks(nt2)), dim3(256), 0, st, tri2, nt2, etab, esz - 1, emult, (const uint8_t*)others, parent,
+                                   probe_limit);
             } else {
-                hipLaunchKernelGGL(cxp_k_edges_claim, dim3(cx_blocks(nt2)), dim3(256), 0, st, tri2, nt2, etab, esz - 1, emult);
+                hipLaunchKernelGGL(cxp_k_edges_claim, dim3(cx_blocks(nt2)), dim3(256), 0, st, tri2, nt2, etab, esz - 1, emult, parent);
                 if (coherent && !cx_debug_knob("CX_LINK_ONE_STEP", 0)) {
                     hipLaunchKernelGGL(cxp_k_edges_link_local, dim3((nt2 + CXP_LINK_BLOCK - 1u) / CXP_LINK_BLOCK), dim3(256), 0, st, tri2, nt2, etab, esz - 1,
                                        emult, parent, others);
@@ -1058,10 +1105,14 @@
                 } else
                     hipLaunchKernelGGL(cxp_k_edges_link, dim3(cx_blocks(nt2)), dim3(256), 0, st, tri2, nt2, etab, esz - 1, emult, parent, coherent ? 1 : 0);
             }
+            if ((rc = cxp_orient_pick(ctx, tri2, nt2, pts2, parent, cmaxx, keys2, cls2, clist, misc, true))) return rc;
+            if (first_table) {
+                CX_HIP(ctx, hipEventSynchronize(S->hev[1]));
+                if (count_entries) fprintf(stderr, "cx edge table: %u entries in %llu slots, %u triangles\n", S->hwords[13], (unsigned long long)esz, nt2);
+                if (S->hwords[12]) { esz = esz_full; continue; }
+            }
             break;
         }
-        uint32_t* clist = S->flags.as<uint32_t>();
-        if ((rc = cxp_orient_pick(ctx, tri2, nt2, pts2, parent, cmaxx, keys2, cls2, clist, misc))) return rc;
         if (shard) {
             uint32_t hb[2] = {0, 0};
             CX_HIP(ctx, hipMemcpyAsync(hb, misc + 6, 2 * sizeof(uint32_t), hipMemcpyDeviceToHost, st));
@@ -1075,7 +1126,6 @@
             uint32_t* label4 = label1 + n1;
             uint8_t* open = cls + 2 * (size_t)nt;
             CX_HIP(ctx, hipMemsetAsync(open, 0, nt2, st));
-            CX_HIP(ctx, hipMemsetAsync(misc + 8, 0, 3 * sizeof(uint32_t), st));
             if (nb) {
                 const u64 key_offset = ((u64)ctx->origin[0] * (u64)shard->plane) << 3;
                 hipLaunchKernelGGL(cxp_k_shard_boundary, dim3(cx_blocks(nt2)), dim3(256), 0, st, cls2, told, tprio3, parent, nt2, key_offset, misc + 8,
@@ -1089,9 +1139,11 @@
             if (h2[0] != n1 || h2[1] != n4 || h2[2] > nb) { ctx->err = "sharded Level 1: boundary lists do not add up"; return CX_ERR_HIP; }
             S->shard.n1 = (uint32_t)n1; S->shard.n4 = (uint32_t)n4; S->shard.ncand = h2[2];
         }
-        if ((rc = cxp_orient_decide(ctx, tri2, nt2, pts2, parent, cmaxx, clist, misc, !shard, &ncomp))) return rc;
+        S->hwords[3] = 0;
+        if ((rc = cxp_orient_decide(ctx, tri2, nt2, pts2, parent, cmaxx, clist, misc, !shard, S->hwords + 3))) return rc;
         if (!shard) { S->orient_live = true; S->orient_nt = nt2; }
         CX_HIP(ctx, hipStreamSynchronize(st));
+        ncomp = S->hwords[3];
     } else if (shard) {
         S->shard.n1 = 0; S->shard.n4 = 0; S->shard.ncand = 0;
     }
@@ -1135,8 +1187,7 @@
         hipLaunchKernelGGL(cxp_k_shard_own_alive, dim3(cx_blocks(nt2)), dim3(256), 0, st, cls2, nt2, alive);
         CX_HIP(ctx, hipMemsetAsync(used, 0, (size_t)nv2, st));
         hipLaunchKernelGGL(cxp_k_mark_used8, dim3(cx_blocks(nt2)), dim3(256), 0, st, (const int32_t*)tri2, (const uint8_t*)alive, nt2, used);
-        hipLaunchKernelGGL(cxp_k_me_count, dim3(nbv), dim3(256), 0, st, (const uint8_t*)used, nv2, voff);
-        hipLaunchKernelGGL(cxp_k_me_count, dim3(nbt), dim3(256), 0, st, (const uint8_t*)alive, nt2, toff);
+        hipLaunchKernelGGL(cxp_k_me_count2, dim3(nbv + nbt), dim3(256), 0, st, (const uint8_t*)used, nv2, voff, nbv, (const uint8_t*)alive, nt2, toff);
         hipLaunchKernelGGL(cxp_k_scan_sums2, dim3(2), dim3(1024), 0, st, voff, nbv, misc + 1, toff, nbt, misc + 2);
         uint32_t h[3];
         CX_HIP(ctx, hipMemcpyAsync(h, misc + 1, 3 * sizeof(uint32_t), hipMemcpyDeviceToHost, st));
@@ -1296,10 +1347,8 @@
     if (nv && nt && (edge_crossings || march_mesh) && coherent) {
         if ((rc = S->ever.grow(ctx, 2 * (size_t)nv + 64))) return rc;
         ever = S->ever.as<uint8_t>();
-        CX_HIP(ctx, hipMemsetAsync(ever, 0, nv, st));
     }
     if (nv && nt) {
-        hipLaunchKernelGGL(cxp_k_tri_prio, dim3(cx_blocks(nt)), dim3(256), 0, st, tri, prio, nt, tprio3);
         cxp_weld_params W;
         for (int a = 0; a < 3; a++) W.ex[a] = std::trunc((10000 * 1.0) / corner[a]);
         W.thr = 0.0;
@@ -1312,16 +1361,16 @@
         if ((rc = S->tvals.grow(ctx, wsz * sizeof(u64)))) return rc;
         hipLaunchKernelGGL(cxp_k_fill64, dim3(2048), dim3(256), 0, st, S->tkeys.as<u64>(), (size_t)wsz, CXD_EMPTY);
         hipLaunchKernelGGL(cxp_k_fill64, dim3(2048), dim3(256), 0, st, S->tvals.as<u64>(), (size_t)wsz, (u64)0);
+        uint8_t* involved = (coherent && !cx_debug_knob("CX_DEDUPE_ALL", 0)) ? moved : nullptr;
         hipLaunchKernelGGL(cxp_k_weld_insert, dim3(cx_blocks(nv)), dim3(256), 0, st, pts, prio, nv, W, S->tkeys.as<u64>(), S->tvals.as<u64>(), wsz - 1, vkeep);
-        hipLaunchKernelGGL(cxp_k_weld_lookup, dim3(cx_blocks(nv)), dim3(256), 0, st, pts, nv, W, S->tkeys.as<u64>(), S->tvals.as<u64>(), wsz - 1, rep, vkeep, prio);
-        uint8_t* involved = (coherent && !cx_debug_knob("CX_DEDUPE_ALL", 0)) ? moved : nullptr;
-        if (involved) CX_HIP(ctx, hipMemsetAsync(involved, 0, nv, st));
-        hipLaunchKernelGGL(cxp_k_remap, dim3(cx_blocks(nt)), dim3(256), 0, st, tri, alive, nt, rep, (const u64*)nullptr, involved, ever);
+        hipLaunchKernelGGL(cxp_k_weld_lookup, dim3(cx_blocks(nv)), dim3(256), 0, st, pts, nv, W, S->tkeys.as<u64>(), S->tvals.as<u64>(), wsz - 1, rep, vkeep, prio,
+                           S->parent.as<u64>(), involved, ever);
+        hipLaunchKernelGGL(cxp_k_remap, dim3(cx_blocks(nt)), dim3(256), 0, st, tri, alive, nt, rep, (const u64*)nullptr, involved, ever, (const uint32_t*)prio, tprio3);
         const u64 tsz = involved ? cxp_edge_table_size(nt) : cx_table_size(nt);
         hipLaunchKernelGGL(cxp_k_fill64, dim3(2048), dim3(256), 0, st, S->tkeys.as<u64>(), (size_t)tsz, CXD_EMPTY);
         hipLaunchKernelGGL(cxp_k_dedupe_insert, dim3(cx_blocks(nt)), dim3(256), 0, st, tri, tprio3, alive, nt, S->tkeys.as<u64>(), tsz - 1, (const uint8_t*)involved);
         hipLaunchKernelGGL(cxp_k_dedupe_resolve, dim3(cx_blocks(nt)), dim3(256), 0, st, tri, alive, nt, S->tkeys.as<u64>(), tsz - 1, (const uint8_t*)involved);
-        CX_HIP(ctx, hipMemsetAsync(misc + 4, 0, 2 * sizeof(uint32_t), st));
+        CX_HIP(ctx, hipMemsetAsync(misc + 3, 0, 11 * sizeof(uint32_t), st));
         hipLaunchKernelGGL(cxp_k_count_alive, dim3(std::min(cx_blocks(nt), 1024u)), dim3(256), 0, st, alive, nt, misc + 4);
         if (smooth > 0.0) {
             const u64 esz = cx_table_size((size_t)nt * 3);
@@ -1342,19 +1391,16 @@
             hipLaunchKernelGGL(cxp_k_smooth_apply, dim3(cx_blocks(nv)), dim3(256), 0, st, pts, sum, cnt, nv, smooth);
         }
         u64* parent = S->parent.as<u64>();
-        hipLaunchKernelGGL(cxp_k_iota64, dim3(cx_blocks(nv)), dim3(256), 0, st, parent, nv);
         CX_HIP(ctx, hipMemsetAsync(moved, 0, nv, st));
         hipLaunchKernelGGL(cxp_k_tiny, dim3(cx_blocks(nt)), dim3(256), 0, st, tri, alive, nt, pts, 1.0 / corner[0], 1.0 / corner[1],
                            1.0 / corner[2], 1e-4, parent, prio, moved);
-        hipLaunchKernelGGL(cxp_k_move, dim3(cx_blocks(nv)), dim3(256), 0, st, pts, pts, parent, moved, nv);
+        if ((rc = S->flags.grow(ctx, (size_t)(nv + nt + 16) * sizeof(uint32_t)))) return rc;
+        hipLaunchKernelGGL(cxp_k_move, dim3(cx_blocks(nv)), dim3(256), 0, st, pts, pts, parent, moved, nv, do_clean ? S->parent2.as<u64>() : (u64*)nullptr,
+                           S->flags.as<uint8_t>());
         hipLaunchKernelGGL(cxp_k_count_alive, dim3(std::min(cx_blocks(nt), 1024u)), dim3(256), 0, st, alive, nt, misc + 5);
-        uint32_t h[2];
-        CX_HIP(ctx, hipMemcpyAsync(h, misc + 4, 2 * sizeof(uint32_t), hipMemcpyDeviceToHost, st));
-        CX_HIP(ctx, hipStreamSynchronize(st));
-        counts[2] = h[0]; counts[3] = h[1];
     }
     return cxp_clean_orient(ctx, S, nv, nt, do_clean, true, tprio3, counts, coherent,
-                            (coherent && nv && nt && !cx_debug_knob("CX_DEDUPE_ALL", 0)) ? moved : nullptr, shard, ever);
+                            (coherent && nv && nt && !cx_debug_knob("CX_DEDUPE_ALL", 0)) ? moved : nullptr, shard, ever, nv && nt);
 }
 
 extern "C" int cx_postprocess3d_ex(cx_ctx* ctx, uint32_t flags, double smooth, int64_t* out_counts) {
```

Measured after the change: 455,800, median of 2. About the same (-0.1%).
